# imisumi/software-path-tracer

Measured on AMD Instinct MI355X. Metric: Msamples/sec (whole node), 1920x1080 x 8-bounce Cornell box, higher is better.
Workload: dtype f32

## Files before the change

include/spt.h:

```cpp
#ifndef SPT_H
#define SPT_H

#include <stddef.h>
#include <stdint.h>

#ifdef __cplusplus
extern "C" {
#endif

#define SPT_ABI_VERSION 3

typedef enum spt_status {
    SPT_OK = 0,
    SPT_ERR_INVALID = -1,
    SPT_ERR_HIP = -2,
    SPT_ERR_NO_DEVICE = -3,
    SPT_ERR_NO_SCENE = -4,
    SPT_ERR_NOT_CONFIGURED = -5,
    SPT_ERR_CAPACITY = -6
} spt_status;


typedef enum spt_prim_type {
    SPT_PRIM_SPHERE = 0,
// ... 111 lines not shown
int spt_configure(spt_ctx* ctx, const spt_config* cfg);
int spt_reset(spt_ctx* ctx);
int spt_get_frame_count(const spt_ctx* ctx, uint32_t* frame_count);

int spt_render(spt_ctx* ctx, uint32_t first_frame, uint32_t n_frames);
int spt_synchronize(spt_ctx* ctx);

int spt_shard_pixels(const spt_ctx* ctx, uint64_t* n_pixels);
int spt_read_accum(spt_ctx* ctx, float* host_rgba);
int spt_accum_device_ptr(spt_ctx* ctx, void** dptr, size_t* bytes);
int spt_copy_accum_device(spt_ctx* ctx, void* dst);
int spt_resolve_rgba8(spt_ctx* ctx, uint32_t frame_count, uint32_t* host_out);
int spt_resolve_rgba8_exposure(spt_ctx* ctx, uint32_t frame_count, float exposure, uint32_t* host_out);
int spt_register_host_output(spt_ctx* ctx, void* host_out, size_t bytes);
int spt_render_resolve_rgba8(spt_ctx* ctx, uint32_t first_frame, uint32_t n_frames, uint32_t frame_count,
                             float exposure, uint32_t* host_out);
int spt_assemble_rows(spt_ctx* ctx, const void* gathered, void* out);

#define SPT_CAMERA_JITTER 1u
typedef struct spt_camera {
    float origin[3], u[3], v[3], w[3];
    uint32_t flags;
    uint32_t reserved[3];
} spt_camera;
int spt_set_camera(spt_ctx* ctx, const spt_camera* camera);
int spt_camera_look_at(const float eye[3], const float target[3], const float up[3], float vfov_degrees,
                       spt_camera* out);
int spt_camera_ray(const spt_camera* camera, uint32_t width, uint32_t height, uint32_t x, uint32_t y,
                   float jx, float jy, float o[3], float d[3]);

typedef struct spt_lens {
    float radius;
    float focus_distance;
    uint32_t reserved[2];
} spt_lens;
int spt_set_camera_lens(spt_ctx* ctx, const spt_lens* lens);
int spt_camera_lens_ray(const spt_camera* camera, const spt_lens* lens, uint32_t width, uint32_t height,
                        uint32_t x, uint32_t y, float jx, float jy, float u1, float u2, float o[3], float d[3]);
int spt_camera_focus_at_hit(const spt_camera* camera, uint32_t width, uint32_t height, uint32_t x, uint32_t y,
                            float jx, float jy, float t, float* focus_distance);

typedef enum spt_material_kind { SPT_MAT_DIFFUSE = 0, SPT_MAT_METAL = 1, SPT_MAT_DIELECTRIC = 2 } spt_material_kind;
typedef struct spt_material_model {
    uint32_t kind;
    float    param;
    uint32_t reserved[2];
} spt_material_model;
int spt_set_material_models(spt_ctx* ctx, const spt_material_model* models, uint32_t n);
int spt_bsdf_sample(const spt_material_model* model, const float d[3], const float n[3], int entering,
                    uint32_t flags, uint32_t* rng, float dir_out[3], int* transmitted, int* absorbed);

int spt_render_features(spt_ctx* ctx);
int spt_read_features(spt_ctx* ctx, float* feat_a, float* feat_b, float* albedo);
int spt_features_device_ptr(spt_ctx* ctx, void** feat_a, void** feat_b, void** albedo, size_t* bytes);

typedef struct spt_denoise_params {
    uint32_t levels;
    float    sigma_color;
    float    sigma_plane;
    uint32_t normal_power_log2;
    uint32_t reserved[4];
} spt_denoise_params;
int spt_denoise_params_default(spt_denoise_params* out);
int spt_denoise(spt_ctx* ctx, uint32_t frame_count, const spt_denoise_params* params);
int spt_set_denoise_form(spt_ctx* ctx, int form);
int spt_read_denoised(spt_ctx* ctx, float* host_rgba);
int spt_denoised_device_ptr(spt_ctx* ctx, void** dptr, size_t* bytes);
int spt_resolve_denoised_rgba8(spt_ctx* ctx, float exposure, uint32_t* host_out);
int spt_atrous_host(const float* rgba, const float* feat_a, const float* feat_b, uint32_t width, uint32_t height,
                    const spt_denoise_params* params, float* out);

int spt_set_env_map(spt_ctx* ctx, const float* rgba, uint32_t width, uint32_t height);
int spt_env_octa_from_equirect(const float* src_rgb, uint32_t src_width, uint32_t src_height, float* dst_rgba,
                               uint32_t dst_width, uint32_t dst_height);

enum spt_profile {
    SPT_PROFILE_EVENTS = 1,
    SPT_PROFILE_COUNTERS = 2,
    SPT_PROFILE_SPAN = 4
};
int spt_set_profiling(spt_ctx* ctx, int mode);
int spt_get_stats(spt_ctx* ctx, spt_stats* out);
int spt_stats_clear(spt_ctx* ctx);

#define SPT_COMM_ID_BYTES 128
int spt_comm_available(void);
int spt_comm_unique_id(uint8_t id[SPT_COMM_ID_BYTES]);
int spt_comm_init(spt_ctx* ctx, const uint8_t id[SPT_COMM_ID_BYTES], int n_ranks, int rank);
int spt_gather_image(spt_ctx* ctx, void* root_image);
int spt_gather_image_overlapped(spt_ctx* ctx, void* root_image);
int spt_gather_wait(spt_ctx* ctx);
int spt_comm_destroy(spt_ctx* ctx);

typedef struct spt_tuning {
    int32_t fused;
    uint32_t tail_bounce;
    int32_t persistent;
    int32_t frame_kernel;
    uint32_t chunks_per_wave;
    uint32_t px_shift;
    uint32_t subqueues;
    uint32_t bvh_max_leaf;
    uint32_t bvh_bins;
    int32_t specialize;
    int32_t view_cache;
    int32_t split_streams;
} spt_tuning;
int spt_set_tuning(spt_ctx* ctx, const spt_tuning* tuning);

int spt_specialize_scene(spt_ctx* ctx);
int spt_compile_flat_kernels(const spt_prim* prims, uint32_t n_prims, int env_map, char* log, size_t log_bytes);

typedef enum spt_scene_id {
    SPT_SCENE_C1_SPHERE_GROUND = 0,
    SPT_SCENE_APP_DEFAULT = 1,
    SPT_SCENE_CORNELL = 2,
    SPT_SCENE_BUNNYLIKE = 3,
    SPT_SCENE_INTERIOR_1M = 4
} spt_scene_id;
int spt_build_scene(uint32_t scene_id, spt_prim* prims, uint32_t* n_prims,
                    spt_material* mats, uint32_t* n_mats, spt_env* env);

#ifdef __cplusplus
}
#endif
#endif
```

software-path-tracer_amd/__init__.py:

```python
from __future__ import annotations

import ctypes
import enum
import os
from typing import Optional, Sequence, Tuple

import numpy as np

_HERE = os.path.dirname(os.path.abspath(__file__))
LIB_PATH = os.environ.get("SPT_LIB_PATH") or os.path.join(_HERE, "libspt_hip.so")
RENDER_LIB_PATH = os.path.join(_HERE, "libspt_render.so")

SPT_OK = 0
SPT_ERR = {
    -1: "SPT_ERR_INVALID",
    -2: "SPT_ERR_HIP",
    -3: "SPT_ERR_NO_DEVICE",
    -4: "SPT_ERR_NO_SCENE",
    -5: "SPT_ERR_NOT_CONFIGURED",
    -6: "SPT_ERR_CAPACITY",
}

PRIM_SPHERE, PRIM_QUAD, PRIM_TRIANGLE = 0, 1, 2
FLAG_ABS_FLOAT = 1
# ... 33 lines not shown
class SptEnv(ctypes.Structure):
    _fields_ = [("sky_enabled", ctypes.c_uint32), ("horizon", ctypes.c_float * 3), ("zenith", ctypes.c_float * 3)]


class SptConfig(ctypes.Structure):
    _fields_ = [
        ("width", ctypes.c_uint32),
        ("height", ctypes.c_uint32),
        ("max_bounces", ctypes.c_uint32),
        ("rr_depth", ctypes.c_uint32),
        ("flags", ctypes.c_uint32),
        ("shard_rank", ctypes.c_uint32),
        ("shard_count", ctypes.c_uint32),
        ("frames_in_flight", ctypes.c_uint32),
    ]


class SptCamera(ctypes.Structure):
    _fields_ = [
        ("origin", ctypes.c_float * 3),
        ("u", ctypes.c_float * 3),
        ("v", ctypes.c_float * 3),
        ("w", ctypes.c_float * 3),
        ("flags", ctypes.c_uint32),
        ("reserved", ctypes.c_uint32 * 3),
    ]


class SptLens(ctypes.Structure):
    _fields_ = [
        ("radius", ctypes.c_float),
        ("focus_distance", ctypes.c_float),
        ("reserved", ctypes.c_uint32 * 2),
    ]


CAMERA_JITTER = 1
SPT_MAX_BOUNCES = 32


class SptStats(ctypes.Structure):
    _fields_ = [
        ("frames", ctypes.c_uint64),
        ("paths", ctypes.c_uint64),
        ("segments", ctypes.c_uint64 * SPT_MAX_BOUNCES),
        ("segments_total", ctypes.c_uint64),
        ("passes", ctypes.c_uint64),
        ("extend_launches", ctypes.c_uint64),
        ("extend_ms", ctypes.c_double),
        ("extend_segments", ctypes.c_uint64),
        ("shade_launches", ctypes.c_uint64),
        ("shade_ms", ctypes.c_double),
        ("other_ms", ctypes.c_double),
        ("extend_ms_bounce", ctypes.c_double * SPT_MAX_BOUNCES),
        ("shade_ms_bounce", ctypes.c_double * SPT_MAX_BOUNCES),
        ("bvh_nodes", ctypes.c_uint64),
        ("scene_bytes", ctypes.c_uint64),
        ("radiance_updates", ctypes.c_uint64 * SPT_MAX_BOUNCES),
        ("tail_ms", ctypes.c_double),
        ("tail_launches", ctypes.c_uint64),
        ("tail_bounce", ctypes.c_uint64),
        ("fused", ctypes.c_uint64),
        ("persistent_ms", ctypes.c_double),
        ("persistent_launches", ctypes.c_uint64),
        ("schedule", ctypes.c_uint64),
        ("lane_slots", ctypes.c_uint64),
        ("lane_busy", ctypes.c_uint64),
        ("bvh_node_visits", ctypes.c_uint64),
        ("prim_tests", ctypes.c_uint64),
        ("flat_fast_path", ctypes.c_uint64),
        ("specialized", ctypes.c_uint64),
        ("shadow_rays", ctypes.c_uint64),
        ("emitters", ctypes.c_uint64),
        ("stack_bytes", ctypes.c_uint64),
        ("stack_need", ctypes.c_uint64),
        ("stalled_waves", ctypes.c_uint64),
        ("view_cached", ctypes.c_uint64),
        ("view_live_pixels", ctypes.c_uint64),
        ("flat_pairs", ctypes.c_uint64),
        ("flat_pair_second_passes", ctypes.c_uint64),
        ("view_split", ctypes.c_uint64),
        ("flat_sphere_second_passes", ctypes.c_uint64),
    ]

    def as_dict(self) -> dict:
        d = {}
        for k, _ in self._fields_:
            v = getattr(self, k)
            d[k] = list(v) if isinstance(v, ctypes.Array) else v
        return d


EXPORTED_SYMBOLS = (
    "spt_abi_version", "spt_device_count", "spt_create", "spt_destroy", "spt_last_error", "spt_set_stream",
    "spt_set_scene", "spt_configure", "spt_reset", "spt_get_frame_count", "spt_render", "spt_synchronize",
    "spt_shard_pixels", "spt_read_accum", "spt_accum_device_ptr", "spt_copy_accum_device", "spt_resolve_rgba8",
    "spt_resolve_rgba8_exposure", "spt_register_host_output", "spt_render_resolve_rgba8", "spt_assemble_rows",
    "spt_set_profiling", "spt_get_stats", "spt_stats_clear", "spt_build_scene",
    "spt_set_env_map", "spt_env_octa_from_equirect",
    "spt_comm_available", "spt_comm_unique_id", "spt_comm_init", "spt_gather_image", "spt_gather_image_overlapped", "spt_gather_wait",
    "spt_comm_destroy", "spt_set_tuning",
    "spt_specialize_scene", "spt_compile_flat_kernels", "spt_update_prims",
    "spt_set_camera", "spt_camera_look_at", "spt_camera_ray",
    "spt_set_camera_lens", "spt_camera_lens_ray", "spt_camera_focus_at_hit",
    "spt_set_material_models", "spt_bsdf_sample",
    "spt_render_features", "spt_read_features", "spt_features_device_ptr",
    "spt_denoise_params_default", "spt_denoise", "spt_set_denoise_form", "spt_read_denoised", "spt_denoised_device_ptr",
    "spt_resolve_denoised_rgba8", "spt_atrous_host",
)
COMM_ID_BYTES = 128


class SptTuning(ctypes.Structure):
    _fields_ = [
        ("fused", ctypes.c_int32),
        ("tail_bounce", ctypes.c_uint32),
        ("persistent", ctypes.c_int32),
        ("frame_kernel", ctypes.c_int32),
        ("chunks_per_wave", ctypes.c_uint32),
        ("px_shift", ctypes.c_uint32),
        ("subqueues", ctypes.c_uint32),
        ("bvh_max_leaf", ctypes.c_uint32),
        ("bvh_bins", ctypes.c_uint32),
        ("specialize", ctypes.c_int32),
        ("view_cache", ctypes.c_int32),
        ("split_streams", ctypes.c_int32),
    ]

    def __init__(self, **kw):
        super().__init__(fused=-1, persistent=-1, frame_kernel=-1)
        for k, v in kw.items():
            if k not in dict(self._fields_):
                raise TypeError(f"unknown spt_tuning field {k}")
            setattr(self, k, v)


class DenoiseParams(ctypes.Structure):
    _fields_ = [
        ("levels", ctypes.c_uint32),
        ("sigma_color", ctypes.c_float),
        ("sigma_plane", ctypes.c_float),
        ("normal_power_log2", ctypes.c_uint32),
        ("reserved", ctypes.c_uint32 * 4),
    ]

    def __init__(self, **kw):
        super().__init__()
        rc = load_library().spt_denoise_params_default(ctypes.byref(self))
        if rc != SPT_OK:
            raise SptError(f"spt_denoise_params_default -> {SPT_ERR.get(rc, rc)}")
        for k, v in kw.items():
            if k not in dict(self._fields_):
                raise TypeError(f"unknown spt_denoise_params field {k}")
            setattr(self, k, v)


_lib: Optional[ctypes.CDLL] = None


class SptError(RuntimeError):
    pass


def load_library(path: str = LIB_PATH) -> ctypes.CDLL:
    global _lib
    if _lib is not None:
        return _lib
    if not os.path.exists(path):
        raise SptError(f"libspt_hip.so not built at {path} (run `make` or __graft_entry__.build())")
    lib = ctypes.CDLL(path)
    P, U32, I = ctypes.c_void_p, ctypes.c_uint32, ctypes.c_int
    sig = {
        "spt_abi_version": ([], I),
        "spt_device_count": ([ctypes.POINTER(I)], I),
        "spt_create": ([ctypes.POINTER(P), I], I),
        "spt_destroy": ([P], None),
        "spt_last_error": ([P], ctypes.c_char_p),
        "spt_set_stream": ([P, P], I),
        "spt_set_scene": ([P, P, U32, P, U32, ctypes.POINTER(SptEnv)], I),
        "spt_configure": ([P, ctypes.POINTER(SptConfig)], I),
        "spt_reset": ([P], I),
        "spt_get_frame_count": ([P, ctypes.POINTER(U32)], I),
        "spt_render": ([P, U32, U32], I),
        "spt_synchronize": ([P], I),
        "spt_shard_pixels": ([P, ctypes.POINTER(ctypes.c_uint64)], I),
        "spt_read_accum": ([P, P], I),
        "spt_accum_device_ptr": ([P, ctypes.POINTER(P), ctypes.POINTER(ctypes.c_size_t)], I),
        "spt_copy_accum_device": ([P, P], I),
        "spt_resolve_rgba8": ([P, U32, P], I),
        "spt_resolve_rgba8_exposure": ([P, U32, ctypes.c_float, P], I),
        "spt_register_host_output": ([P, P, ctypes.c_size_t], I),
        "spt_render_resolve_rgba8": ([P, U32, U32, U32, ctypes.c_float, P], I),
        "spt_assemble_rows": ([P, P, P], I),
        "spt_set_profiling": ([P, I], I),
        "spt_set_env_map": ([P, P, U32, U32], I),
        "spt_env_octa_from_equirect": ([P, U32, U32, P, U32, U32], I),
        "spt_get_stats": ([P, ctypes.POINTER(SptStats)], I),
        "spt_stats_clear": ([P], I),
        "spt_build_scene": ([U32, P, ctypes.POINTER(U32), P, ctypes.POINTER(U32), ctypes.POINTER(SptEnv)], I),
        "spt_comm_available": ([], I),
        "spt_comm_unique_id": ([P], I),
        "spt_comm_init": ([P, P, I, I], I),
        "spt_gather_image": ([P, P], I),
        "spt_gather_image_overlapped": ([P, P], I),
        "spt_gather_wait": ([P], I),
        "spt_comm_destroy": ([P], I),
        "spt_set_tuning": ([P, ctypes.POINTER(SptTuning)], I),
        "spt_specialize_scene": ([P], I),
        "spt_update_prims": ([P, P, P, U32], I),
        "spt_compile_flat_kernels": ([P, U32, I, ctypes.c_char_p, ctypes.c_size_t], I),
        "spt_set_camera": ([P, ctypes.POINTER(SptCamera)], I),
        "spt_camera_look_at": ([ctypes.POINTER(ctypes.c_float), ctypes.POINTER(ctypes.c_float),
                                ctypes.POINTER(ctypes.c_float), ctypes.c_float, ctypes.POINTER(SptCamera)], I),
        "spt_camera_ray": ([ctypes.POINTER(SptCamera), U32, U32, U32, U32, ctypes.c_float, ctypes.c_float,
                            ctypes.POINTER(ctypes.c_float), ctypes.POINTER(ctypes.c_float)], I),
        "spt_set_camera_lens": ([P, ctypes.POINTER(SptLens)], I),
        "spt_camera_lens_ray": ([ctypes.POINTER(SptCamera), ctypes.POINTER(SptLens), U32, U32, U32, U32,
                                 ctypes.c_float, ctypes.c_float, ctypes.c_float, ctypes.c_float,
                                 ctypes.POINTER(ctypes.c_float), ctypes.POINTER(ctypes.c_float)], I),
        "spt_camera_focus_at_hit": ([ctypes.POINTER(SptCamera), U32, U32, U32, U32, ctypes.c_float, ctypes.c_float,
                                     ctypes.c_float, ctypes.POINTER(ctypes.c_float)], I),
        "spt_set_material_models": ([P, P, U32], I),
        "spt_bsdf_sample": ([P, ctypes.POINTER(ctypes.c_float), ctypes.POINTER(ctypes.c_float), I, U32,
                             ctypes.POINTER(U32), ctypes.POINTER(ctypes.c_float), ctypes.POINTER(I),
                             ctypes.POINTER(I)], I),
        "spt_render_features": ([P], I),
        "spt_read_features": ([P, P, P, P], I),
        "spt_features_device_ptr": ([P, ctypes.POINTER(P), ctypes.POINTER(P), ctypes.POINTER(P),
                                     ctypes.POINTER(ctypes.c_size_t)], I),
        "spt_denoise_params_default": ([ctypes.POINTER(DenoiseParams)], I),
        "spt_denoise": ([P, U32, ctypes.POINTER(DenoiseParams)], I),
        "spt_set_denoise_form": ([P, I], I),
        "spt_read_denoised": ([P, P], I),
        "spt_denoised_device_ptr": ([P, ctypes.POINTER(P), ctypes.POINTER(ctypes.c_size_t)], I),
        "spt_resolve_denoised_rgba8": ([P, ctypes.c_float, P], I),
        "spt_atrous_host": ([P, P, P, U32, U32, ctypes.POINTER(DenoiseParams), P], I),
    }
    for name, (args, res) in sig.items():
        if os.environ.get("SPT_LIB_PATH") and not hasattr(lib, name):
            continue
        fn = getattr(lib, name)
        fn.argtypes = args
        fn.restype = res
    _lib = lib
    return lib


def _ptr(a: np.ndarray) -> ctypes.c_void_p:
    return ctypes.c_void_p(a.ctypes.data) if a.size else ctypes.c_void_p(0)


def reference_env(sky: bool = True) -> SptEnv:
    e = SptEnv()
    e.sky_enabled = 1 if sky else 0
    e.horizon[:] = (1.0, 1.0, 1.0)
    e.zenith[:] = (0.5, 0.7, 1.0)
    return e


def env_octa_from_equirect(equirect_rgb: np.ndarray, width: int, height: int) -> np.ndarray:
    src = np.ascontiguousarray(equirect_rgb, dtype=np.float32)
    dst = np.zeros((height, width, 4), dtype=np.float32)
    rc = load_library().spt_env_octa_from_equirect(src.ctypes.data, src.shape[1], src.shape[0], dst.ctypes.data,
                                                   width, height)
    if rc != 0:
        raise SptError(f"spt_env_octa_from_equirect: {rc}")
    return dst


def synthetic_env_map(size: int = 512, seed: int = 0x5eed) -> np.ndarray:
    h, w = size // 2, size
    theta = (np.arange(h, dtype=np.float64) + 0.5) / h * np.pi
    phi = (np.arange(w, dtype=np.float64) + 0.5) / w * 2 * np.pi - np.pi
    th, ph = np.meshgrid(theta, phi, indexing="ij")
    y = np.cos(th)
    base = np.stack([0.6 + 0.4 * y, 0.7 + 0.3 * y, 1.0 + 0.2 * y], axis=-1)
    sun = np.exp(-((th - 0.6) ** 2 + (ph - 0.8) ** 2) / 0.002)[..., None] * np.array([40.0, 36.0, 30.0])
    ground = (y < 0)[..., None] * np.array([-0.3, -0.35, -0.5])
    noise = np.random.default_rng(seed).uniform(0.0, 0.05, size=(h, w, 1))
    equirect = np.maximum(base + sun + ground + noise, 0.0).astype(np.float32)
# ... 295 lines not shown
        self._env_keep = a
        self._check(self.lib.spt_set_env_map(self.h, a.ctypes.data, a.shape[1], a.shape[0]), "spt_set_env_map")

    def set_camera(self, cam: Optional[SptCamera]) -> None:
        self._check(self.lib.spt_set_camera(self.h, ctypes.byref(cam) if cam is not None else None), "spt_set_camera")
        self._camera = SptCamera.from_buffer_copy(cam) if cam is not None else None

    def set_camera_lens(self, radius=None, focus_distance: float = 1.0) -> None:
        if radius is None:
            self._check(self.lib.spt_set_camera_lens(self.h, None), "spt_set_camera_lens")
            return
        lens = _lens(radius, focus_distance)
        self._check(self.lib.spt_set_camera_lens(self.h, ctypes.byref(lens)), "spt_set_camera_lens")

    def focus_at(self, x: int, y: int) -> Optional[float]:
        if self._camera is None:
            raise SptError("focus_at needs a camera (set_camera)")
        w, h = self.width, self.height
        rank, count = int(self.cfg.shard_rank), max(1, int(self.cfg.shard_count))
        if not (0 <= x < w and 0 <= y < h) or y % count != rank:
            raise SptError("focus_at: the pixel is outside the image or on another ctx's rows")
        _, feat_b, _ = self.read_features()
        t = float(feat_b.reshape(-1, w, 4)[y // count, x, 3])
        if not np.isfinite(t):
            return None
        j = 0.5 if self._camera.flags & CAMERA_JITTER else 0.0
        return camera_focus_at_hit(self._camera, w, h, x, y, t, j, j)

    def set_material_models(self, models) -> None:
        if models is None:
            self._check(self.lib.spt_set_material_models(self.h, None, 0), "spt_set_material_models")
            return
        m = material_models(models)
        self._check(self.lib.spt_set_material_models(self.h, m.ctypes.data, len(m)), "spt_set_material_models")

    def render_features(self) -> None:
        self._check(self.lib.spt_render_features(self.h), "spt_render_features")

    def read_features(self) -> Tuple[np.ndarray, np.ndarray, np.ndarray]:
        n = self.shard_pixels
        a, b, alb = (np.zeros((n, 4), dtype=np.float32) for _ in range(3))
        self._check(self.lib.spt_read_features(self.h, _ptr(a), _ptr(b), _ptr(alb)), "spt_read_features")
        return a, b, alb

    def features_device_ptr(self) -> Tuple[int, int, int, int]:
        a, b, alb, n = ctypes.c_void_p(), ctypes.c_void_p(), ctypes.c_void_p(), ctypes.c_size_t()
        self._check(self.lib.spt_features_device_ptr(self.h, ctypes.byref(a), ctypes.byref(b), ctypes.byref(alb),
                                                     ctypes.byref(n)), "spt_features_device_ptr")
        return a.value or 0, b.value or 0, alb.value or 0, n.value

    def denoise(self, frame_count: int, params: Optional[DenoiseParams] = None) -> None:
        self._check(self.lib.spt_denoise(self.h, frame_count, ctypes.byref(params) if params is not None else None),
                    "spt_denoise")

    def set_denoise_form(self, form: int) -> None:
        self._check(self.lib.spt_set_denoise_form(self.h, form), "spt_set_denoise_form")

    def read_denoised(self) -> np.ndarray:
        out = np.zeros((self.shard_pixels, 4), dtype=np.float32)
        self._check(self.lib.spt_read_denoised(self.h, _ptr(out)), "spt_read_denoised")
        return out

    def denoised_device_ptr(self) -> Tuple[int, int]:
        p, n = ctypes.c_void_p(), ctypes.c_size_t()
        self._check(self.lib.spt_denoised_device_ptr(self.h, ctypes.byref(p), ctypes.byref(n)), "spt_denoised_device_ptr")
        return p.value or 0, n.value

    def resolve_denoised_rgba8(self, exposure: float = 1.0, out: Optional[np.ndarray] = None) -> np.ndarray:
        if out is None:
            out = np.zeros(self.shard_pixels, dtype=np.uint32)
        elif out.dtype != np.uint32 or not out.flags["C_CONTIGUOUS"] or out.size < self.shard_pixels:
            raise SptError("resolve_denoised_rgba8: out must be a C-contiguous uint32 array of >= shard_pixels")
        self._check(self.lib.spt_resolve_denoised_rgba8(self.h, exposure, _ptr(out)), "spt_resolve_denoised_rgba8")
        return out

    def set_profiling(self, enable, counters: bool = False, span: bool = False) -> None:
        mode = (PROFILE_EVENTS if enable and not span else 0) | (PROFILE_COUNTERS if counters else 0) | \
            (PROFILE_SPAN if span and enable else 0)
        self._check(self.lib.spt_set_profiling(self.h, mode), "spt_set_profiling")

    def stats(self) -> SptStats:
        s = SptStats()
        self._check(self.lib.spt_get_stats(self.h, ctypes.byref(s)), "spt_get_stats")
        return s

    def clear_stats(self) -> None:
        self._check(self.lib.spt_stats_clear(self.h), "spt_stats_clear")


def comm_available() -> bool:
    return load_library().spt_comm_available() == SPT_OK


def comm_unique_id() -> bytes:
    buf = ctypes.create_string_buffer(COMM_ID_BYTES)
    rc = load_library().spt_comm_unique_id(buf)
    if rc != SPT_OK:
        raise SptError(f"spt_comm_unique_id -> {SPT_ERR.get(rc, rc)}")
    return buf.raw


def device_count() -> int:
    lib = load_library()
    n = ctypes.c_int()
    lib.spt_device_count(ctypes.byref(n))
    return n.value


class BackendType(enum.IntEnum):

    CPU_EMBREE = 0
    GPU_OPTIX = 1
    GPU_METAL = 2
    GPU_HIP = 3


class RenderSettings:

    def __init__(self):
        self._width, self._height = 512, 512
        self._progressive = True
        self._spp, self._max_bounces, self._rr_depth = 64, 8, 3
        self._exposure = 1.0
        self._dirty = True

    def _set(self, name, value):
        if getattr(self, name) != value:
            setattr(self, name, value)
            self._dirty = True

    def setResolution(self, width: int, height: int) -> None:
        if (self._width, self._height) != (width, height):
            self._width, self._height = width, height
            self._dirty = True

    def setProgressive(self, v: bool) -> None:
        self._set("_progressive", v)

    def setSamplesPerPixel(self, v: int) -> None:
        self._set("_spp", v)

    def setMaxBounces(self, v: int) -> None:
        self._set("_max_bounces", v)

    def setRussianRouletteDepth(self, v: int) -> None:
        self._set("_rr_depth", v)

    def setExposure(self, v: float) -> None:
        self._set("_exposure", v)

    def getProgressive(self) -> bool:
        return self._progressive

    def getWidth(self) -> int:
        return self._width

    def getHeight(self) -> int:
        return self._height

    def getSamplesPerPixel(self) -> int:
        return self._spp

    def getMaxBounces(self) -> int:
        return self._max_bounces

    def getRussianRouletteDepth(self) -> int:
# ... 187 lines not shown
```

software-path-tracer_amd/csrc/spt_capi.hip:

```cpp
#include <dlfcn.h>
#include <hip/hip_runtime.h>
#include <rccl/rccl.h>

#include <algorithm>
#include <cmath>
#include <cstdio>
#include <cstdlib>
#include <cstring>
#include <string>
#include <vector>

#include "scene.h"
#include "spt.h"
#include "spt_denoise.h"
#include "spt_device.h"
#include "spt_jit.h"
#include "spt_kernels.h"
#include "spt_launch_plan.h"

using namespace spt;

static_assert(kBvhStackMax == kBvhStackEntries, "scene.h and spt_kernels.h stack bounds");
static_assert(kMatDiffuse == SPT_MAT_DIFFUSE && kMatMetal == SPT_MAT_METAL && kMatDielectric == SPT_MAT_DIELECTRIC,
              "spt.h spt_material_kind and spt_device.h model_kind");
static_assert(sizeof(spt_material_model) == 16, "spt_material_model is 16 bytes");
static_assert(sizeof(spt_denoise_params) == 32, "spt_denoise_params is 32 bytes");

namespace {

struct DevTree {
    std::vector<uint8_t> bytes;
    uint32_t stack_need = 0, stack_tb = 0;
};
template <int W, class Q, class QuantFn>
DevTree make_dev_tree(const std::vector<BvhNode>& bin, QuantFn quantize) {
    static_assert(sizeof(Q) == kDevNodeBytes, "device node record size");
    DevTree t;
    std::vector<BvhNodeW<W>> wide;
    collapse_bvh_w<W>(bin, wide);
    if (wide.empty()) return t;
    t.stack_need = bvh_w_stack_need<W>(wide, 0u);
    t.stack_tb = bvh_stack_t0_bits(bvh_w_max_ref<W>(wide));
    std::vector<Q> q;
    quantize(wide, q);
    t.bytes.resize(sizeof(Q) * q.size());
    std::memcpy(t.bytes.data(), q.data(), t.bytes.size());
    return t;
}
DevTree device_tree(const std::vector<BvhNode>& bin) { return make_dev_tree<4, BvhNodeQ>(bin, quantize_bvh4); }

struct EventPair {
    hipEvent_t a = nullptr, b = nullptr;
    int kind = 0;
    uint32_t bounce = 0;
    uint32_t launches = 1;
    hipEvent_t a2 = nullptr, b2 = nullptr;
};

struct ViewHalf {
    hipStream_t stream = nullptr;
    hipEvent_t done = nullptr;
    uint16_t* cost = nullptr;
    uint32_t* order = nullptr;
    uint64_t order_key = 0;
    uint32_t* work = nullptr;
    uint32_t work_parity = 0;
};

}

struct spt_ctx {
    int device = -1;
    hipStream_t own_stream = nullptr;
    hipStream_t user_stream = nullptr;
    ViewHalf half[2];
    hipEvent_t fork_ev = nullptr;
    bool stream_dirty = true;
    int32_t split_streams = 0;
    bool last_view_split = false;
    bool accum_shared = false;
    std::string err;
    uint32_t cu_count = 256;

    float4* d_prims = nullptr;
    float4* d_mats = nullptr;
    float4* d_nodes = nullptr;
    float4* d_env = nullptr;
    float4* d_emit = nullptr;
    uint32_t n_emit = 0;
    uint32_t n_emit_spheres = 0;
    uint32_t env_w = 0, env_h = 0;
    uint32_t n_prims = 0, n_nodes = 0, n_mats = 0;
    uint32_t n_dev_nodes = 0;
    void* bvh_stack = nullptr;
    uint32_t bvh_stack_need = 0;
    uint32_t bvh_stack_stride = 0;
    uint32_t bvh_stack_tb = 1;
    spt_env env{};
    bool has_scene = false;
    uint32_t flat_ends = 0;
    uint32_t flat_rect = 0;
    uint32_t flat_pairs = 0;
    bool fast_div = false;
    uint64_t scene_bytes = 0;
    uint64_t stack_bytes = 0;

    spt_config cfg{};
    bool configured = false;
    uint32_t rows = 0;
    uint32_t pixels = 0;
    uint32_t frames_per_pass = 1;
    uint32_t n_sub = 0;
    uint32_t sub_cap = 0;

    float4* q_o[2] = {nullptr, nullptr};
    float4* q_d[2] = {nullptr, nullptr};
    float4* q_t[2] = {nullptr, nullptr};
    float2* hit = nullptr;
    float4* radiance = nullptr;
    float4* accum = nullptr;
    float2* hit_cache = nullptr;
    bool hit_cache_valid = false;
    uint16_t* chunk_cost = nullptr;
    uint32_t* chunk_order = nullptr;
    uint64_t chunk_order_key = 0;
    float4* view_live = nullptr;
    float4* view_const = nullptr;
    uint32_t* view_counts = nullptr;
    uint32_t view_n[2] = {0, 0};
    bool view_valid = false;
    bool view_no_memory = false;
    int32_t view_cache = 0;
    bool last_view_cached = false;
    bool frame_lists = false;
    uint4* live_rec = nullptr;
    uint32_t* sky_pix = nullptr;
    uint32_t* list_counts = nullptr;
    uint32_t live_pixels = 0;
    uint32_t* counts = nullptr;
    unsigned long long* totals = nullptr;
    uint32_t* work = nullptr;
    uint32_t work_parity = 0;
    uint32_t chunks_per_wave = 0;
    uint32_t px_shift = 0;
    uint32_t* resolved = nullptr;
    void* out_host = nullptr;
    void* out_dev = nullptr;
    size_t out_bytes = 0;
    float fuse_frames = 0.0f, fuse_exposure = 1.0f;
    bool fused = false;

    uint32_t frame_count = 0;

    float4* feat_a = nullptr;
    float4* feat_b = nullptr;
    float4* feat_albedo = nullptr;
    bool feat_valid = false;
    uint32_t* d_mat_map = nullptr;
    float4* dn[2] = {nullptr, nullptr};
    int dn_result = -1;
    int dn_form = -1;

// ... 290 lines not shown
    if (!c->span_open) return SPT_OK;
    c->span_open = false;
    return end_event(c, c->span_ev);
}

bool schedule_fused(const spt_ctx* c) {
    if (c->cfg.flags & (SPT_FLAG_SPLIT_KERNELS | SPT_FLAG_SORTED_RAYS)) return false;
    if (c->fused_override >= 0) return c->fused_override != 0;
    return c->n_nodes == 0;
}

constexpr uint32_t kPersistentMaxFrames = 1024;

bool schedule_persistent(const spt_ctx* c, uint32_t n_frames) {
    if (c->cfg.max_bounces == 0) return false;
    if (c->cfg.flags & (SPT_FLAG_SPLIT_KERNELS | SPT_FLAG_WAVEFRONT | SPT_FLAG_SORTED_RAYS)) return false;
    if (c->persistent_override >= 0) return c->persistent_override != 0;
    return n_frames >= SPT_PERSISTENT_MIN_FRAMES;
}

bool schedule_frame(const spt_ctx* c) {
    if (c->cfg.max_bounces == 0) return false;
    if (c->cfg.flags & (SPT_FLAG_SPLIT_KERNELS | SPT_FLAG_WAVEFRONT | SPT_FLAG_SORTED_RAYS)) return false;
    if (c->frame_override >= 0) return c->frame_override != 0;
    if (c->persistent_override >= 0) return c->persistent_override != 0;
    return true;
}

uint32_t schedule_tail(const spt_ctx* c) {
    if (c->tail_override) return c->tail_override;
    return c->n_nodes == 0 ? 3u : kMaxBounces;
}

void next_work_set(spt_ctx* c, PassParams& p) {
    p.work = c->work + c->work_parity * kWorkWords;
    p.work_next = c->work + (c->work_parity ^ 1u) * kWorkWords;
    c->work_parity ^= 1u;
}

static uint64_t flat_jit_key(const spt_ctx* c) {
    const uint64_t shape = flat_shape_key(c->flat_ends, c->n_prims, c->flat_rect, c->flat_pairs);
    if (!c->configured) return shape;
    const uint32_t flags = (c->cfg.flags & ~spt::kFlagFastDiv) | (c->fast_div ? spt::kFlagFastDiv : 0u);
    return jit_config_key(shape, c->cfg.max_bounces, c->cfg.rr_depth, c->env.sky_enabled ? 1u : 0u, flags, c->has_camera);
}

static uint32_t sphere_emitters(const std::vector<DevEmitter>& emit) {
    uint32_t k = 0;
    for (const DevEmitter& e : emit) {
        uint32_t kind;
        std::memcpy(&kind, &e.base[3], 4);
        k += kind == 2u ? 1u : 0u;
    }
    return k;
}
static bool nee_active(const spt_ctx* c) { return c->configured && (c->cfg.flags & SPT_FLAG_NEE) && c->n_emit != 0u; }

static uint32_t camera_mode(const spt_ctx* c) {
    return ((c->camera.flags & SPT_CAMERA_JITTER) ? kCamJitter : kCamPosed) | (c->has_lens ? kCamLens : 0u);
}
static CameraLens lens_scalars(const spt_camera& cam, const spt_lens& lens) {
    auto len = [](const float v[3]) {
        return std::sqrt(((double)v[0] * v[0] + (double)v[1] * v[1]) + (double)v[2] * v[2]);
    };
    const double lu = len(cam.u), lv = len(cam.v);
    return CameraLens{lu > 0.0 ? (float)((double)lens.radius / lu) : 0.0f,
                      lv > 0.0 ? (float)((double)lens.radius / lv) : 0.0f, lens.focus_distance};
}
static int write_camera_record(spt_ctx* c) {
    SPT_HIP(c, hipSetDevice(c->device));
    SPT_HIP(c, hipStreamSynchronize(on_stream(c)));
    if (!c->d_camera) SPT_HIP(c, hipMalloc(&c->d_camera, 4 * sizeof(float4)));
    const spt_camera& cam = c->camera;
    const CameraLens l = c->has_lens ? lens_scalars(cam, c->lens) : CameraLens{0.0f, 0.0f, 0.0f};
    const uint32_t mode = camera_mode(c);
    float4 rec[4] = {make_float4(cam.origin[0], cam.origin[1], cam.origin[2], 0.0f),
                     make_float4(cam.u[0], cam.u[1], cam.u[2], l.a), make_float4(cam.v[0], cam.v[1], cam.v[2], l.b),
                     make_float4(cam.w[0], cam.w[1], cam.w[2], l.f)};
    std::memcpy(&rec[0].w, &mode, sizeof(mode));
    SPT_HIP(c, hipMemcpy(c->d_camera, rec, sizeof(rec), hipMemcpyHostToDevice));
    return SPT_OK;
}

static void prefetch_flat(const spt_ctx* c) {
    if (!(c->has_scene && c->configured && c->n_prims && c->n_nodes == 0 && c->specialize == 0)) return;
    const uint64_t key = flat_jit_key(c);
    const JitKindList kinds = jit_kinds_of_scene(nee_active(c), c->d_env ? 1 : 0);
    for (int i = 0; i < kinds.n; ++i) jit_prefetch(kinds.k[i].kind, kinds.k[i].env, key);
}

PassParams base_params(spt_ctx* c) {
    PassParams p{};
    p.prims = c->d_prims;
    p.mats = c->d_mats;
    p.nodes = c->d_nodes;
    p.n_prims = c->n_prims;
    p.n_mats = c->n_mats;
    p.n_nodes = c->n_nodes;
    p.n_dev_nodes = c->n_dev_nodes;
    p.sky_enabled = c->env.sky_enabled ? 1u : 0u;
    p.flags = (c->cfg.flags & ~spt::kFlagFastDiv) | (c->fast_div ? spt::kFlagFastDiv : 0u);
    p.flat_ends = c->flat_ends;
    for (int a = 0; a < 3; ++a) {
        p.bin_lo[a] = c->scene_lo[a];
        const float ext = c->scene_hi[a] - c->scene_lo[a];
        p.bin_scale[a] = ext > 0.0f ? 8.0f / ext : 0.0f;
    }
    p.ray_keys = c->ray_keys;
    p.ray_perm = c->ray_perm;
    p.ray_bins = c->ray_bins;
    p.ray_cursor = c->ray_cursor;
    p.jit_shape = (c->n_prims && c->n_nodes == 0 && c->specialize >= 0) ? flat_jit_key(c) : 0ull;
    p.jit_wait = c->specialize > 0 ? 1u : 0u;
    p.horizon = make_float4(c->env.horizon[0], c->env.horizon[1], c->env.horizon[2], 0.0f);
    p.zenith = make_float4(c->env.zenith[0], c->env.zenith[1], c->env.zenith[2], 0.0f);
    p.env = c->d_env;
    p.env_w = c->env_w;
    p.env_h = c->env_h;
    p.width = c->cfg.width;
    p.height = c->cfg.height;
    p.shard_rank = c->cfg.shard_rank;
    p.shard_count = c->cfg.shard_count;
    p.shard_pixels = c->pixels;
    p.inv_h = 1.0f / (float)c->cfg.height;
    p.inv_w = 1.0f / (float)c->cfg.width;
    p.aspect = (float)c->cfg.width / (float)c->cfg.height;
    p.max_bounces = c->cfg.max_bounces;
    p.rr_depth = c->cfg.rr_depth;
    p.n_sub = c->n_sub;
    p.sub_cap = c->sub_cap;
    for (int k = 0; k < 2; ++k) p.q[k] = QueueBufs{c->q_o[k], c->q_d[k], c->q_t[k]};
    p.hit = c->hit;
    p.radiance = c->radiance;
    p.accum = c->accum;
    p.counts = c->counts;
    p.totals = c->totals;
    p.cu_count = c->cu_count;
    p.chunks_per_wave = c->chunks_per_wave ? c->chunks_per_wave
                                           : ((c->n_nodes != 0 && c->n_prims <= 256u * 1024u) ? 4u : 2u);
    p.px_shift = c->px_shift;
    p.stack = c->bvh_stack;
    p.stack_need = c->bvh_stack_need;
    p.stack_stride = c->bvh_stack_stride;
    p.stack_tb = c->bvh_stack_tb;
    p.nee = NeeParams{c->d_emit, nee_active(c) ? c->n_emit : 0u, c->n_emit_spheres};
    if (c->has_camera) {
        p.cam_mode = camera_mode(c);
        p.cam_pose = c->d_camera;
    }
    p.bsdf = c->bsdf ? 1u : 0u;
    return p;
}

float model_word(const spt_material_model& m) {
    if (m.kind == SPT_MAT_METAL) return -std::fabs(m.param);
    return m.kind == SPT_MAT_DIELECTRIC ? m.param : 0.0f;
}
const char* model_error(const spt_material_model& m) {
    if (m.reserved[0] | m.reserved[1]) return "material model: reserved must be 0";
    if (!std::isfinite(m.param)) return "material model: non-finite parameter";
    if (m.kind == SPT_MAT_DIFFUSE) return m.param == 0.0f ? nullptr : "material model: a DIFFUSE parameter must be 0";
    if (m.kind == SPT_MAT_METAL) return m.param >= 0.0f && m.param <= 1.0f ? nullptr : "material model: fuzz outside [0, 1]";
    if (m.kind == SPT_MAT_DIELECTRIC) return m.param > 0.0f ? nullptr : "material model: index of refraction not > 0";
    return "material model: unknown kind";
}
int upload_materials(spt_ctx* c) {
    std::vector<DevMaterial> dm = c->h_dm;
    bool bsdf = false;
    if (!c->h_models.empty())
        for (size_t i = 0; i < dm.size(); ++i) {
// ... 390 lines not shown
        SPT_HIP(c, hipMalloc(&c->hit_cache, sizeof(float2) * std::max<size_t>(pixels, 1)));
        SPT_HIP(c, hipMalloc(&c->chunk_cost, sizeof(uint16_t) * std::max<size_t>(pixels, 1)));
        SPT_HIP(c, hipMalloc(&c->chunk_order, sizeof(uint32_t) * std::max<size_t>(pixels, 1)));
        if (kFrameHitCache >= 2) {
            SPT_HIP(c, hipMalloc(&c->live_rec, sizeof(uint4) * std::max<size_t>(pixels, 1)));
            SPT_HIP(c, hipMalloc(&c->sky_pix, sizeof(uint32_t) * std::max<size_t>(pixels, 1)));
            SPT_HIP(c, hipMalloc(&c->list_counts, sizeof(uint32_t) * (2 + (pixels + kBlock - 1) / kBlock)));
        }
        SPT_HIP(c, hipMalloc(&c->resolved, sizeof(uint32_t) * std::max<size_t>(pixels, 1)));
    }
    c->hit_cache_valid = false;
    c->feat_valid = false;
    c->dn_result = -1;
    c->chunk_order_key = 0;
    c->view_valid = false;
    const size_t qn = (size_t)cap * c->n_sub;
    if ((cfg->flags & SPT_FLAG_SORTED_RAYS) && qn && !c->ray_perm) {
        SPT_HIP(c, hipMalloc(&c->ray_keys, sizeof(uint16_t) * qn));
        SPT_HIP(c, hipMalloc(&c->ray_perm, sizeof(uint32_t) * qn));
        SPT_HIP(c, hipMalloc(&c->ray_bins, sizeof(uint32_t) * 4096));
        SPT_HIP(c, hipMalloc(&c->ray_cursor, sizeof(uint32_t) * 4097));
        SPT_HIP(c, hipMemset(c->ray_bins, 0, sizeof(uint32_t) * 4096));
    }
    c->configured = true;
    prefetch_flat(c);
    return spt_reset(c);
}

int spt_reset(spt_ctx* c) {
    if (!c) return SPT_ERR_INVALID;
    if (!c->configured) return fail(c, SPT_ERR_NOT_CONFIGURED, "spt_reset before spt_configure");
    SPT_HIP(c, hipSetDevice(c->device));
    SPT_HIP(c, hipMemsetAsync(c->accum, 0, sizeof(float4) * std::max<size_t>(c->pixels, 1), on_stream(c)));
    c->frame_count = 0;
    return SPT_OK;
}

int spt_get_frame_count(const spt_ctx* c, uint32_t* fc) {
    if (!c || !fc) return SPT_ERR_INVALID;
    *fc = c->frame_count;
    return SPT_OK;
}

static int build_view_lists(spt_ctx* c, const PassParams& p) {
    const size_t pixels = std::max<size_t>(c->pixels, 1);
    if (!c->view_live) {
        const size_t blocks = (pixels + kBlock - 1) / kBlock;
        if (hipMalloc(&c->view_live, sizeof(float4) * 3 * pixels) != hipSuccess ||
            hipMalloc(&c->view_const, sizeof(float4) * pixels) != hipSuccess ||
            hipMalloc(&c->view_counts, sizeof(uint32_t) * (2 + blocks)) != hipSuccess) {
            (void)hipGetLastError();
            free_dev(c->view_live);
            free_dev(c->view_const);
            free_dev(c->view_counts);
            c->view_no_memory = true;
            return SPT_OK;
        }
    }
    launch_view_lists(p, c->view_live, c->view_const, c->view_counts, c->view_counts + 2, on_stream(c));
    SPT_HIP(c, hipGetLastError());
    SPT_HIP(c, hipMemcpyAsync(c->view_n, c->view_counts, 2 * sizeof(uint32_t), hipMemcpyDeviceToHost, on_stream(c)));
    SPT_HIP(c, hipStreamSynchronize(on_stream(c)));
    c->view_valid = true;
    for (ViewHalf& h : c->half) h.order_key = 0;
    return SPT_OK;
}


static bool half_buffers(spt_ctx* c) {
    const size_t n = (size_t)c->pixels / 2u + 64u;
    for (ViewHalf& h : c->half) {
        if (h.cost && h.order) continue;
        if (hipMalloc(&h.cost, sizeof(uint16_t) * n) != hipSuccess || hipMalloc(&h.order, sizeof(uint32_t) * n) != hipSuccess) {
            (void)hipGetLastError();
            free_dev(h.cost);
            free_dev(h.order);
            return false;
        }
        h.order_key = 0;
    }
    return true;
}

static int launch_paths_split(spt_ctx* c, PassParams p, const ViewPlan& whole, bool launched[2]) {
    const ViewSplit sp = make_view_split(whole.n_live, whole.n_const, 1u << kMaxChunkShift);
    EventPair span_ev;
    if (c->profiling && c->span && begin_persistent(c, span_ev) != SPT_OK) return SPT_ERR_HIP;
    if (c->stream_dirty || c->accum_shared) {
        SPT_HIP(c, hipEventRecord(c->fork_ev, c->user_stream));
        for (ViewHalf& h : c->half) SPT_HIP(c, hipStreamWaitEvent(h.stream, c->fork_ev, 0));
        c->stream_dirty = false;
    }
    if (!c->chunks_per_wave) p.chunks_per_wave = 0u;
    const bool timed = c->profiling && !c->span;
    EventPair ev[2];
    int n_ev = 0;
    int rc = SPT_OK;
    for (uint32_t h = 0; h < 2u && rc == SPT_OK; ++h) {
        if (view_half_empty(sp, h)) continue;
        ViewHalf& vh = c->half[h];
        const ViewPlan view{whole.live + 3u * (size_t)sp.live_at[h], whole.constant + sp.const_at[h],
                            sp.live_at[h + 1] - sp.live_at[h], sp.const_at[h + 1] - sp.const_at[h], 0u};
        p.work = vh.work + vh.work_parity * kWorkWords;
        p.work_next = vh.work + (vh.work_parity ^ 1u) * kWorkWords;
        vh.work_parity ^= 1u;
        p.chunk_cost = vh.cost;
        p.chunk_order = vh.order;
        p.chunk_order_key = &vh.order_key;
        if (timed) {
            if (take_events(c, ev[n_ev], 4) != SPT_OK) return SPT_ERR_HIP;
            ++n_ev;
            if (hipEventRecord(ev[n_ev - 1].a, vh.stream) != hipSuccess) rc = fail(c, SPT_ERR_HIP, "k_paths (split): hipEventRecord");
        }
        c->last_specialized = launch_paths(p, c->counters, vh.stream, &view, h + 1u);
        launched[h] = true;
        const hipError_t le = hipGetLastError();
        if (le != hipSuccess) {
            vh.order_key = 0;
            rc = fail(c, SPT_ERR_HIP, std::string("k_paths (split): ") + hipGetErrorString(le));
        }
        if (timed && hipEventRecord(ev[n_ev - 1].b, vh.stream) != hipSuccess) rc = fail(c, SPT_ERR_HIP, "k_paths (split): hipEventRecord");
    }
    c->last_pairs = c->last_specialized ? flat_shape_pairs(p.jit_shape) : 0u;
    if (rc != SPT_OK) {
        for (int i = 0; i < n_ev; ++i) c->free_events.push_back(ev[i]);
        for (ViewHalf& h : c->half) h.order_key = 0;
        return rc;
    }
    if (n_ev) {
        if (n_ev == 2) {
            ev[0].a2 = ev[1].a;
            ev[0].b2 = ev[1].b;
        }
        c->pending.push_back(ev[0]);
        if (c->pending.size() >= 4096) return flush_events(c);
    }
    return SPT_OK;
}

static int join_halves(spt_ctx* c, bool launched[2]) {
    int rc = SPT_OK;
    for (uint32_t h = 0; h < 2u; ++h) {
        if (!launched[h]) continue;
        launched[h] = false;
        hipError_t e = hipEventRecord(c->half[h].done, c->half[h].stream);
        if (e == hipSuccess) e = hipStreamWaitEvent(c->user_stream, c->half[h].done, 0);
        if (e != hipSuccess) rc = fail(c, SPT_ERR_HIP, std::string("k_paths (split) join: ") + hipGetErrorString(e));
    }
    return rc;
}

static int render_persistent(spt_ctx* c, PassParams& p, uint32_t first_frame, uint32_t n_frames, bool launched[2]) {
    uint32_t done = 0;
    while (done < n_frames) {
        const uint32_t f = std::min(kPersistentMaxFrames, n_frames - done);
        p.first_frame = first_frame + done;
        p.n_frames = f;
        p.n_paths = f * c->pixels;
        const bool view_scene = c->view_cache >= 0 && view_lists_scene(p);
        const ViewPlan view{c->view_live, c->view_const, c->view_n[0], c->view_n[1], 0u};
        const bool view_on = view_scene && c->view_valid;
        if (view_on && split_call_wanted(c->split_streams, c->view_n[0], n_frames, kPersistentMaxFrames) && half_buffers(c)) {
            c->last_view_cached = c->last_view_split = true;
            const int rc = launch_paths_split(c, p, view, launched);
            if (rc != SPT_OK) return rc;
            done += f;
            c->passes++;
            continue;
        }
        if (join_halves(c, launched) != SPT_OK) return SPT_ERR_HIP;
        c->last_view_split = false;
        EventPair ev;
        if (begin_persistent(c, ev) != SPT_OK) return SPT_ERR_HIP;
        next_work_set(c, p);
        p.chunk_cost = c->chunk_cost;
        p.chunk_order = c->chunk_order;
        p.chunk_order_key = &c->chunk_order_key;
        c->last_specialized = launch_paths(p, c->counters, on_stream(c), view_on ? &view : nullptr);
        c->last_pairs = c->last_specialized ? flat_shape_pairs(p.jit_shape) : 0u;
        c->last_view_cached = view_on;
        const hipError_t le = hipGetLastError();
        if (le != hipSuccess) c->chunk_order_key = 0;
        if (end_persistent(c, ev) != SPT_OK) {
            c->chunk_order_key = 0;
            return SPT_ERR_HIP;
        }
        SPT_HIP(c, le);
        if (view_scene && !c->view_valid && !c->view_no_memory && build_view_lists(c, p) != SPT_OK) return SPT_ERR_HIP;
        done += f;
        c->passes++;
    }
    return SPT_OK;
}

int spt_render(spt_ctx* c, uint32_t first_frame, uint32_t n_frames) {
    if (!c) return SPT_ERR_INVALID;
    if (!c->has_scene) return fail(c, SPT_ERR_NO_SCENE, "Scene not set before rendering");
    if (!c->configured) return fail(c, SPT_ERR_NOT_CONFIGURED, "spt_render before spt_configure");
    if (c->sub_alloc != c->n_sub) return fail(c, SPT_ERR_NOT_CONFIGURED, "spt_set_tuning(subqueues) takes effect at spt_configure");
    SPT_HIP(c, hipSetDevice(c->device));
    if (c->pixels == 0 || n_frames == 0) {
        c->frame_count += n_frames;
        return SPT_OK;
    }
    PassParams p = base_params(c);
    uint32_t done = 0;
    if (schedule_persistent(c, n_frames)) {
        c->last_schedule = SPT_SCHEDULE_PERSISTENT;
        bool launched[2] = {false, false};
        const int rc = render_persistent(c, p, first_frame, n_frames, launched);
        const std::string err = c->err;
        const int joined = join_halves(c, launched);
        if (rc != SPT_OK) {
            c->err = err;
            return rc;
        }
        if (joined != SPT_OK) return joined;
        c->frames += n_frames;
        c->paths += (uint64_t)n_frames * c->pixels;
        c->frame_count += n_frames;
        return SPT_OK;
    }
    if (schedule_frame(c)) {
        c->last_schedule = SPT_SCHEDULE_FRAME;
        for (; done < n_frames; ++done) {
            p.first_frame = first_frame + done;
            p.n_frames = 1;
            p.n_paths = c->pixels;
            EventPair ev;
            if (begin_persistent(c, ev) != SPT_OK) return SPT_ERR_HIP;
            next_work_set(c, p);
            p.hit_cache = c->hit_cache;
            p.live_rec = c->live_rec;
            p.sky_pix = c->sky_pix;
            p.list_counts = c->list_counts;
            const bool jitter = cam_per_path(p.cam_mode) || p.bsdf != 0u;
            p.hit_mode = frame_hit_mode(p, c->hit_cache_valid, c->frame_lists);
            p.live_pixels = c->live_pixels;
            if (c->fuse_frames != 0.0f && done + 1u == n_frames) {
                p.rgba = (uint32_t*)c->out_dev;
                p.rgba_frames = c->fuse_frames;
                p.rgba_exposure = c->fuse_exposure;
                c->fused = true;
            }
            c->last_specialized = launch_frame(p, c->counters, on_stream(c));
            c->last_pairs = c->last_specialized ? flat_shape_pairs(p.jit_shape) : 0u;
            if (end_persistent(c, ev) != SPT_OK) return SPT_ERR_HIP;
            SPT_HIP(c, hipGetLastError());
            if (!c->hit_cache_valid) c->frame_lists = false;
            if (!jitter && !c->hit_cache_valid && frame_lists_scene(p, c->counters)) {
                launch_hit_lists(p, c->list_counts + 2, on_stream(c));
                SPT_HIP(c, hipGetLastError());
                SPT_HIP(c, hipMemcpyAsync(&c->live_pixels, c->list_counts, sizeof(uint32_t), hipMemcpyDeviceToHost,
                                          on_stream(c)));
                SPT_HIP(c, hipStreamSynchronize(on_stream(c)));
                c->frame_lists = c->pixels - c->live_pixels >= c->pixels / kFrameListsMinSkyDiv;
            }
            if (!jitter) c->hit_cache_valid = true;
            c->passes++;
        }
        c->frames += n_frames;
// ... 596 lines not shown
            float* o = dst + 4ull * ((size_t)iy * dw + ix);
            o[0] = t[0];
            o[1] = t[1];
            o[2] = t[2];
            o[3] = 1.0f;
        }
    }
    return SPT_OK;
}

int spt_set_profiling(spt_ctx* c, int mode) {
    if (!c) return SPT_ERR_INVALID;
    SPT_HIP(c, hipSetDevice(c->device));
    const bool span = (mode & SPT_PROFILE_SPAN) != 0;
    if (!span && close_span(c) != SPT_OK) return SPT_ERR_HIP;
    if (!(mode & (SPT_PROFILE_EVENTS | SPT_PROFILE_SPAN)) && flush_events(c) != SPT_OK) return SPT_ERR_HIP;
    c->profiling = (mode & (SPT_PROFILE_EVENTS | SPT_PROFILE_SPAN)) != 0;
    c->span = span;
    const bool counters = (mode & SPT_PROFILE_COUNTERS) != 0;
    if (counters != c->counters) c->hit_cache_valid = false;
    if (counters != c->counters) c->view_valid = false;
    c->counters = counters;
    return SPT_OK;
}

int spt_get_stats(spt_ctx* c, spt_stats* out) {
    if (!c || !out) return SPT_ERR_INVALID;
    SPT_HIP(c, hipSetDevice(c->device));
    SPT_HIP(c, hipStreamSynchronize(on_stream(c)));
    if (flush_events(c) != SPT_OK) return SPT_ERR_HIP;
    unsigned long long tot[kTotals];
    SPT_HIP(c, hipMemcpy(tot, c->totals, sizeof(tot), hipMemcpyDeviceToHost));
    std::memset(out, 0, sizeof(*out));
    out->frames = c->frames;
    out->paths = c->paths;
    out->passes = c->passes;
    for (uint32_t b = 0; b < kMaxBounces && b < SPT_MAX_BOUNCES; ++b) {
        out->segments[b] = tot[b];
        out->segments_total += tot[b];
        out->radiance_updates[b] = tot[kMaxBounces + b];
    }
    out->extend_launches = c->ext_launches;
    out->extend_ms = c->ext_ms;
    out->extend_segments = c->ext_launches ? out->segments_total : 0;
    out->shade_launches = c->shade_launches;
    out->shade_ms = c->shade_ms;
    out->other_ms = c->other_ms;
    out->tail_ms = c->tail_ms;
    out->tail_launches = c->tail_launches;
    out->tail_bounce = schedule_tail(c);
    out->fused = schedule_fused(c) ? 1u : 0u;
    out->persistent_ms = c->persist_ms;
    out->persistent_launches = c->persist_launches;
    out->schedule = c->last_schedule;
    out->lane_slots = tot[2 * kMaxBounces];
    out->lane_busy = tot[2 * kMaxBounces + 1];
    out->bvh_node_visits = tot[2 * kMaxBounces + 2];
    out->prim_tests = tot[2 * kMaxBounces + 3];
    out->flat_fast_path = (c->fast_div && c->n_prims <= kFlatSceneMax) ? 1u : 0u;
    out->specialized = c->last_specialized ? 1u : 0u;
    for (uint32_t b = 0; b < kMaxBounces && b < SPT_MAX_BOUNCES; ++b) {
        out->extend_ms_bounce[b] = c->ext_ms_b[b];
        out->shade_ms_bounce[b] = c->shade_ms_b[b];
    }
    out->bvh_nodes = c->n_nodes;
    out->scene_bytes = c->scene_bytes;
    out->shadow_rays = tot[kTotShadow];
    out->emitters = c->n_emit;
    out->stack_bytes = c->stack_bytes;
    out->stack_need = c->bvh_stack_need;
    out->stalled_waves = tot[kTotStalled];
    out->view_cached = c->last_view_cached ? 1u : 0u;
    out->view_live_pixels = c->view_valid ? c->view_n[0] : 0u;
    out->flat_pairs = c->last_specialized ? c->last_pairs : 0u;
    out->flat_pair_second_passes = tot[kTotPairSecond];
    out->flat_sphere_second_passes = tot[kTotSphereSecond];
    out->view_split = c->last_view_split ? 1u : 0u;
    if (tot[kTotStalled])
        return fail(c, SPT_ERR_HIP, "k_paths: " + std::to_string(tot[kTotStalled]) +
                                        " wave(s) stopped at the step bound with frames unaccumulated (a bug)");
    return SPT_OK;
}

int spt_stats_clear(spt_ctx* c) {
    if (!c) return SPT_ERR_INVALID;
    SPT_HIP(c, hipSetDevice(c->device));
    SPT_HIP(c, hipStreamSynchronize(on_stream(c)));
    if (flush_events(c) != SPT_OK) return SPT_ERR_HIP;
    SPT_HIP(c, hipMemset(c->totals, 0, sizeof(unsigned long long) * kTotals));
    c->frames = c->paths = c->passes = 0;
    c->ext_launches = c->shade_launches = c->ext_segments = 0;
    c->ext_ms = c->shade_ms = c->other_ms = c->tail_ms = 0.0;
    c->tail_launches = 0;
    c->persist_ms = 0.0;
    c->persist_launches = 0;
    for (uint32_t b = 0; b < kMaxBounces; ++b) c->ext_ms_b[b] = c->shade_ms_b[b] = 0.0;
    return SPT_OK;
}

int spt_specialize_scene(spt_ctx* c) {
    if (!c) return SPT_ERR_INVALID;
    if (!c->has_scene) return fail(c, SPT_ERR_NO_SCENE, "spt_specialize_scene before spt_set_scene");
    if (c->n_prims == 0 || c->n_nodes != 0 || c->specialize < 0) return SPT_OK;
    SPT_HIP(c, hipSetDevice(c->device));
    const uint64_t key = flat_jit_key(c);
    std::string err;
    const JitKindList kinds = jit_kinds_of_scene(nee_active(c), c->d_env ? 1 : 0);
    for (int i = 0; i < kinds.n; ++i)
        if (!jit_function(kinds.k[i].kind, kinds.k[i].env, key, &err))
            return fail(c, SPT_ERR_HIP, ("specialized kernels unavailable (the generic ones run): " + err).c_str());
    return SPT_OK;
}

int spt_compile_flat_kernels(const spt_prim* prims, uint32_t n_prims, int env_map, char* log, size_t log_bytes) {
    if (log && log_bytes) log[0] = 0;
    if ((!prims && n_prims) || n_prims == 0 || n_prims > kFlatSceneMax) return SPT_ERR_INVALID;
    uint32_t n_mats = 1;
    for (uint32_t i = 0; i < n_prims; ++i) n_mats = std::max(n_mats, prims[i].material + 1u);
    std::vector<DevPrim> dp, sorted;
    const char* msg = nullptr;
    if (!prepare_prims(prims, n_prims, n_mats, dp, &msg)) return SPT_ERR_INVALID;
    uint32_t ends[kFlatKinds - 1], flat_ends = 0;
    sort_flat_by_kind(dp, sorted, ends);
    for (uint32_t g = 0; g + 1 < kFlatKinds; ++g) flat_ends |= ends[g] << (6 * g);
    const uint32_t flat_rect = flat_rect_bits(sorted, ends);
    const uint64_t key = flat_shape_key(flat_ends, n_prims, flat_rect, flat_wall_pairs(sorted, ends, flat_rect));
    std::string out;
    const JitKindList kinds = jit_kinds_of_scene(false, env_map ? 1 : 0);
    int built = 0;
    while (built < kinds.n && jit_compile(kinds.k[built].kind, kinds.k[built].env, key, &out)) ++built;
    if (built == kinds.n) return SPT_OK;
    if (log && log_bytes) {
        std::strncpy(log, out.c_str(), log_bytes - 1);
        log[log_bytes - 1] = 0;
    }
    return SPT_ERR_HIP;
}

int spt_set_tuning(spt_ctx* c, const spt_tuning* t) {
    if (!c || !t) return SPT_ERR_INVALID;
    if (t->fused < -1 || t->fused > 1 || t->persistent < -1 || t->persistent > 1 || t->frame_kernel < -1 ||
        t->frame_kernel > 1)
        return fail(c, SPT_ERR_INVALID, "spt_tuning: fused / persistent / frame_kernel must be -1, 0 or 1");
    if (t->px_shift && (t->px_shift < 2 || t->px_shift > 5)) return fail(c, SPT_ERR_INVALID, "spt_tuning: px_shift 2..5");
    if (t->chunks_per_wave > 1024 || t->subqueues > 65536 || t->tail_bounce > kMaxBounces ||
        t->bvh_max_leaf > kBvhMaxLeaf || (t->bvh_bins && (t->bvh_bins < 2 || t->bvh_bins > 64)) ||
        t->specialize < -1 || t->specialize > 1 || t->view_cache < -1 || t->view_cache > 0 || t->split_streams < -1 ||
        t->split_streams > 1)
        return fail(c, SPT_ERR_INVALID, "spt_tuning: value out of range");
    SPT_HIP(c, hipSetDevice(c->device));
    SPT_HIP(c, hipStreamSynchronize(on_stream(c)));
    const uint32_t n_sub = t->subqueues ? t->subqueues : c->cu_count * 12u;
    if (n_sub != c->n_sub) {
        uint32_t* counts = nullptr;
        const size_t bytes = sizeof(uint32_t) * 2 * (kMaxBounces + 1) * n_sub;
        SPT_HIP(c, hipMalloc(&counts, bytes));
        if (hipMemset(counts, 0, bytes) != hipSuccess) {
            (void)hipFree(counts);
            return fail(c, SPT_ERR_HIP, "spt_set_tuning: hipMemset of the sub-queue counters failed");
        }
        free_dev(c->counts);
        c->counts = counts;
        c->n_sub = n_sub;
    }
    c->fused_override = t->fused;
    c->tail_override = t->tail_bounce;
    c->persistent_override = t->persistent;
    c->frame_override = t->frame_kernel;
    c->chunks_per_wave = t->chunks_per_wave;
    c->px_shift = t->px_shift;
    c->bvh_max_leaf = t->bvh_max_leaf;
    c->bvh_bins = t->bvh_bins;
    c->specialize = t->specialize;
    c->view_cache = t->view_cache;
    c->split_streams = t->split_streams;
    return SPT_OK;
}

int spt_comm_available(void) { return rccl().ok ? SPT_OK : SPT_ERR_NO_DEVICE; }

int spt_comm_unique_id(uint8_t id[SPT_COMM_ID_BYTES]) {
    static_assert(sizeof(ncclUniqueId) == SPT_COMM_ID_BYTES, "RCCL unique id size");
    if (!id) return SPT_ERR_INVALID;
    if (!rccl().ok) return SPT_ERR_NO_DEVICE;
    ncclUniqueId u;
    if (rccl().get_unique_id(&u) != ncclSuccess) return SPT_ERR_HIP;
    std::memcpy(id, &u, sizeof(u));
    return SPT_OK;
}

int spt_comm_init(spt_ctx* c, const uint8_t id[SPT_COMM_ID_BYTES], int n_ranks, int rank) {
    if (!c || !id) return SPT_ERR_INVALID;
    if (n_ranks < 1 || rank < 0 || rank >= n_ranks) return fail(c, SPT_ERR_INVALID, "spt_comm_init: rank out of range");
    if (!rccl().ok) return fail(c, SPT_ERR_NO_DEVICE, rccl().err);
    SPT_HIP(c, hipSetDevice(c->device));
    SPT_HIP(c, hipStreamSynchronize(on_stream(c)));
    free_comm(c);
    ncclUniqueId u;
    std::memcpy(&u, id, sizeof(u));
    SPT_NCCL(c, rccl().comm_init_rank(&c->comm, n_ranks, u, rank));
    c->comm_ranks = n_ranks;
    c->comm_rank = rank;
    return SPT_OK;
}

int spt_comm_destroy(spt_ctx* c) {
    if (!c) return SPT_ERR_INVALID;
    SPT_HIP(c, hipSetDevice(c->device));
    SPT_HIP(c, hipStreamSynchronize(on_stream(c)));
    free_comm(c);
    return SPT_OK;
}

namespace {
int gather_check(spt_ctx* c, void* root_image, const char* what, uint32_t& rows_max, size_t& shard_elems) {
    if (!c->configured) return fail(c, SPT_ERR_NOT_CONFIGURED, "not configured");
    if (!c->comm) return fail(c, SPT_ERR_INVALID, std::string(what) + " before spt_comm_init");
    const uint32_t world = c->cfg.shard_count;
    if ((int)world != c->comm_ranks || (int)c->cfg.shard_rank != c->comm_rank)
        return fail(c, SPT_ERR_INVALID, std::string(what) + ": shard_rank / shard_count differ from the communicator's rank / size");
    if (c->comm_rank == 0 && !root_image) return fail(c, SPT_ERR_INVALID, std::string(what) + ": rank 0 needs an output image");
    SPT_HIP(c, hipSetDevice(c->device));
    rows_max = (c->cfg.height + world - 1) / world;
    shard_elems = (size_t)rows_max * c->cfg.width * 4;
    return SPT_OK;
}

int gather_buffer(spt_ctx* c, size_t need) {
    if (c->gather_elems == need) return SPT_OK;
    if (c->gather_pending) SPT_HIP(c, hipStreamWaitEvent(on_stream(c), c->gather_done, 0));
    SPT_HIP(c, hipStreamSynchronize(on_stream(c)));
    free_dev(c->gather_buf);
    if (need) {
        SPT_HIP(c, hipMalloc(&c->gather_buf, sizeof(float) * need));
        SPT_HIP(c, hipMemsetAsync(c->gather_buf, 0, sizeof(float) * need, on_stream(c)));
    }
    c->gather_elems = need;
    return SPT_OK;
}
}

int spt_gather_image(spt_ctx* c, void* root_image) {
    if (!c) return SPT_ERR_INVALID;
    uint32_t rows_max = 0;
    size_t shard_elems = 0;
    int st = gather_check(c, root_image, "spt_gather_image", rows_max, shard_elems);
    if (st != SPT_OK) return st;
    const bool root = c->comm_rank == 0;
    const bool padded = c->rows < rows_max;
    st = gather_buffer(c, root ? shard_elems * c->cfg.shard_count : (padded ? shard_elems : 0));
    if (st != SPT_OK) return st;
    if (c->gather_pending) SPT_HIP(c, hipStreamWaitEvent(on_stream(c), c->gather_done, 0));
    const float4* send = c->accum;
    if (padded && !root) {
        if (c->pixels)
            SPT_HIP(c, hipMemcpyAsync(c->gather_buf, c->accum, sizeof(float4) * c->pixels, hipMemcpyDeviceToDevice, on_stream(c)));
        send = c->gather_buf;
    }
// ... 51 lines not shown
```

software-path-tracer_amd/csrc/spt_jit.h:

```cpp
#pragma once

#include <hip/hip_runtime.h>
#include <stdint.h>

#include <string>
#include <vector>

namespace spt {

enum : int { kJitPaths, kJitFrame, kJitPathsChan, kJitPathsNee, kJitFrameNee, kJitFrameRgba, kJitFrameNeeRgba,
             kJitPathsStats, kJitPathsNeeStats, kJitKinds };
constexpr int kJitCallersEnv = -1;
struct JitKindRow {
    const char* kernel;
    const char* tail;
    int env;
    bool stats;
};
constexpr JitKindRow kJitKindTable[kJitKinds] = {
    {"k_paths", "", kJitCallersEnv},
    {"k_frame", "", kJitCallersEnv},
    {"k_paths", ", 0, true", kJitCallersEnv},
    {"k_paths", ", 0, false, 1", 2},
    {"k_frame", ", false, 1", 2},
    {"k_frame", ", false, 0, true", kJitCallersEnv},
    {"k_frame", ", false, 1, true", 2},
    {"k_paths", "", kJitCallersEnv, true},
    {"k_paths", ", 0, false, 1", 2, true},
};
inline std::string jit_name_expr(int kind, int env, uint64_t shape) {
    const JitKindRow& k = kJitKindTable[kind];
    return std::string("spt::") + k.kernel + (k.stats ? "<true, false, " : "<false, false, ") +
           std::to_string(k.env == kJitCallersEnv ? env : k.env) + ", " + std::to_string((unsigned long long)shape) + "ull" + k.tail + ">";
}

bool jit_compile(int kernel, int env, uint64_t shape, std::string* log, std::vector<char>* code = nullptr);
std::string jit_compiler();
hipFunction_t jit_function(int kernel, int env, uint64_t shape, std::string* err, bool wait = true);
void jit_prefetch(int kernel, int env, uint64_t shape);
bool jit_ready(int kernel, int env, uint64_t shape);

}
```

software-path-tracer_amd/csrc/spt_kernels.h:

```cpp
#pragma once

#ifndef __HIPCC_RTC__
#include <hip/hip_runtime.h>
#include <stdint.h>
#endif

namespace spt {

constexpr uint32_t kBlock = 256;
constexpr uint32_t kChunk = 64;
constexpr uint32_t kMaxBounces = 32;
constexpr uint32_t kFlagFastDiv = 1u << 30;
constexpr uint32_t kTotShadow = 2 * kMaxBounces + 4;
constexpr uint32_t kTotStalled = 2 * kMaxBounces + 5;
constexpr uint32_t kTotPairSecond = 2 * kMaxBounces + 6;
constexpr uint32_t kTotSphereSecond = 2 * kMaxBounces + 7;
constexpr uint32_t kOnePassMax = 4;
constexpr uint32_t kTotals = 2 * kMaxBounces + 8;

constexpr uint32_t kFlagNee = 1u << 4;
struct NeeParams {
    const float4* emit;
    uint32_t n_emit;
    uint32_t spheres;
// ... 59 lines not shown
    uint32_t hit_mode;
    const uint4* live_rec;
    const uint32_t* sky_pix;
    const uint32_t* list_counts;
    uint32_t live_pixels;
    uint32_t* rgba;
    float rgba_frames, rgba_exposure;
    uint16_t* chunk_cost;
    uint32_t* chunk_order;
    uint64_t* chunk_order_key;
    uint32_t cam_mode;
    uint32_t bsdf;
    const float4* cam_pose;
};

constexpr uint32_t kCamReference = 0;
constexpr uint32_t kCamPosed = 1;
constexpr uint32_t kCamJitter = 2;
constexpr uint32_t kCamLens = 4;
__host__ __device__ constexpr bool cam_per_path(uint32_t cam_mode) { return (cam_mode & (kCamJitter | kCamLens)) != 0u; }

constexpr uint64_t kShapeValid = 1ull << 36;
__host__ __device__ constexpr uint64_t flat_shape_key(uint32_t flat_ends, uint32_t n_prims, uint32_t rect_bits = 0u,
                                                      uint32_t pair_bits = 0u) {
    return kShapeValid | (uint64_t)(n_prims & 63u) << 30 | (flat_ends & 0x3fffffffu) | (uint64_t)(rect_bits & 7u) << 53 |
           (uint64_t)(pair_bits & 63u) << 57;
}
__host__ __device__ constexpr uint32_t flat_shape_pairs(uint64_t key, uint32_t ax) {
    return (uint32_t)(key >> (57u + 2u * ax)) & 3u;
}
__host__ __device__ constexpr uint32_t flat_shape_pairs(uint64_t key) {
    return flat_shape_pairs(key, 0u) + flat_shape_pairs(key, 1u) + flat_shape_pairs(key, 2u);
}
__host__ __device__ constexpr uint32_t flat_pair_table_bytes(uint64_t key) {
    return flat_shape_pairs(key) ? 64u * flat_shape_pairs(key) + 16u : 0u;
}
constexpr uint64_t kConfigValid = 1ull << 37;
constexpr uint32_t kFlagAbsFloatBit = 1u;
constexpr uint64_t kConfigCamera = 1ull << 56;
__host__ __device__ constexpr uint64_t jit_config_key(uint64_t shape, uint32_t max_bounces, uint32_t rr_depth,
                                                      uint32_t sky_enabled, uint32_t flags, bool camera = false) {
    if (max_bounces > 63u || rr_depth > 63u) return shape;
    return shape | kConfigValid | (uint64_t)max_bounces << 38 | (uint64_t)rr_depth << 44 |
           (uint64_t)(sky_enabled != 0u) << 50 | (uint64_t)((flags & kFlagAbsFloatBit) != 0u) << 51 |
           (uint64_t)((flags & kFlagFastDiv) != 0u) << 52 | (camera ? kConfigCamera : 0ull);
}

constexpr uint32_t kBvhStackEntry = 4;
constexpr uint32_t kBvhStackEntry8W = 8;
constexpr uint32_t kBvhStackEntryBytes = kBvhStackEntry > kBvhStackEntry8W ? kBvhStackEntry : kBvhStackEntry8W;
inline __host__ __device__ constexpr uint32_t bvh_stack_t0_bits(uint32_t max_ref) {
    uint32_t rb = 0;
    while (rb < 32u && (max_ref >> rb) != 0u) ++rb;
    const uint32_t tb = 32u - rb;
    return tb > 28u ? 28u : tb;
}
struct StackCode {
    uint32_t sh, base, mask;
};
inline __host__ __device__ constexpr StackCode stack_code_params(uint32_t tb) {
    return StackCode{28u - tb, 0x3a800000u >> (28u - tb), (1u << tb) - 1u};
}
inline __host__ __device__ constexpr uint32_t stack_code(uint32_t t0_bits, StackCode c) {
    const uint32_t q = (t0_bits >> c.sh) - c.base;
    return q < c.mask ? q : c.mask;
}
inline __host__ __device__ constexpr uint32_t stack_t0_lower_bits(uint32_t code, StackCode c) {
    return ((code & c.mask) + c.base) << c.sh;
}
constexpr uint32_t kBvhStackEntries = 96;
inline __host__ __device__ constexpr uint32_t bvh_stack_stride(uint32_t need) { return need < 1u ? 1u : (need + 3u) & ~3u; }
constexpr uint32_t kMaxResidentWaves = 8 * 4;
constexpr uint32_t kDevNodeBytes = 64u;

constexpr uint32_t kFrameHitCache = 2;
constexpr uint32_t kFrameListsMinSkyDiv = 4;

constexpr int kBvhSmallWaves = 8;
constexpr uint32_t kFrameTopPrims = 64;
constexpr uint32_t kFrameTopNodes = 64;
constexpr uint32_t kBvhSmall = 256u * 1024u;
constexpr uint32_t kMaxChunkShift = 5;
constexpr uint32_t kMinChunkShift = 0;

struct ChunkPlan {
    uint32_t n[3];
    uint32_t start[3];
    uint32_t shift[3];
    const uint32_t* order;
    uint16_t* cost;
};

constexpr uint32_t kViewSweep = 64;
struct ViewPlan {
    const float4* live;
    const float4* constant;
    uint32_t n_live, n_const;
    uint32_t n_sweep;
};

constexpr uint32_t kFrameRun = 128;
constexpr uint32_t kFrameRunBvh = 64;
constexpr uint32_t kFrameLdsStackMax = 16;
__host__ __device__ constexpr uint32_t frame_chunk(bool bvh) { return bvh ? kFrameRunBvh : kFrameRun; }
constexpr int kFrameWavesSmall = 5;
constexpr uint32_t kFrameSkyPerLane = 4;

constexpr uint32_t kWorkHeads = 8;
constexpr uint32_t kWorkStride = 32;
constexpr uint32_t kWorkWords = kWorkHeads * kWorkStride;

#ifndef __HIPCC_RTC__
void launch_extend(const PassParams& p, uint32_t bounce, hipStream_t s);
void launch_extend_sorted(const PassParams& p, uint32_t bounce, hipStream_t s);
void launch_shade(const PassParams& p, uint32_t bounce, hipStream_t s);
void launch_bounce(const PassParams& p, uint32_t bounce, hipStream_t s);
void launch_trace_tail(const PassParams& p, uint32_t bounce, hipStream_t s);
void launch_accumulate(const PassParams& p, hipStream_t s);
bool launch_paths(const PassParams& p, bool stats, hipStream_t s, const ViewPlan* view = nullptr,
                  uint32_t view_half = 0u);
inline bool view_lists_scene(const PassParams& p) {
    return p.nodes == nullptr && p.n_prims != 0u && !cam_per_path(p.cam_mode) && p.bsdf == 0u;
}
void launch_view_lists(const PassParams& p, float4* live, float4* constant, uint32_t* counts, uint32_t* block_scratch,
                       hipStream_t s);
bool launch_frame(const PassParams& p, bool stats, hipStream_t s);
inline bool frame_small_scene(const PassParams& p, bool stats) {
    return p.nodes != nullptr && !stats && p.nee.n_emit == 0u && p.n_dev_nodes <= kFrameTopNodes &&
           p.n_prims <= kFrameTopPrims && 4u * p.n_prims + 2u * p.n_mats <= 4u * kFrameTopPrims &&
           p.stack_need <= kFrameLdsStackMax;
}
inline bool frame_small_scene_lists(const PassParams& p) {
    return p.shard_pixels / kFrameRunBvh > (uint32_t)kFrameWavesSmall * 4u * p.cu_count;
}
inline bool frame_lists_scene(const PassParams& p, bool stats) {
    if (kFrameHitCache < 2) return false;
    if (frame_small_scene(p, stats)) return frame_small_scene_lists(p);
    return true;
}
void launch_hit_lists(const PassParams& p, uint32_t* block_scratch, hipStream_t s);
void launch_resolve(const float4* accum, uint32_t n, float frames, float exposure, uint32_t* out, hipStream_t s);
void launch_assemble_rows(const float4* gathered, float4* out, uint32_t width, uint32_t height,
                          uint32_t world, uint32_t rows_max, hipStream_t s);

#endif

inline __host__ __device__ uint32_t deal_sub(uint32_t p, uint32_t n_sub) { return (p / kChunk) % n_sub; }
inline __host__ __device__ uint32_t deal_slot(uint32_t p, uint32_t n_sub) {
    return (p / (kChunk * n_sub)) * kChunk + (p % kChunk);
}
inline __host__ __device__ uint32_t dealt_path(uint32_t s, uint32_t i, uint32_t n_sub) {
    return ((i / kChunk) * n_sub + s) * kChunk + (i % kChunk);
}
inline __host__ __device__ uint32_t sub_count_of(uint32_t n, uint32_t s, uint32_t n_sub) {
    const uint32_t per_round = kChunk * n_sub;
    const uint32_t full = (n / per_round) * kChunk;
    const uint32_t rem = n % per_round;
    const uint32_t lo = s * kChunk;
    const uint32_t extra = rem > lo ? (rem - lo < kChunk ? rem - lo : kChunk) : 0u;
    return full + extra;
}
inline uint32_t sub_capacity(uint64_t n_paths, uint32_t n_sub) {
    const uint64_t per_round = (uint64_t)kChunk * n_sub;
    return (uint32_t)(((n_paths + per_round - 1) / per_round) * kChunk);
}

}
```

software-path-tracer_amd/csrc/spt_kernels.hip:

```cpp
#ifndef __HIPCC_RTC__
#include <algorithm>
#endif

#include "spt_device.h"
#include "spt_kernels.h"

namespace spt {

namespace {

__device__ __forceinline__ float isect_any(const float4* __restrict__ prims, uint32_t k, uint32_t type, F3 o, F3 d) {
    if (type == 0u) return isect_sphere(prims[4 * k + 0], o, d, kTNear);
    if (type == 1u) return isect_quad(prims[4 * k + 0], prims[4 * k + 1], prims[4 * k + 2], prims[4 * k + 3], o, d, kTNear);
    return isect_tri(prims[4 * k + 0], prims[4 * k + 1], prims[4 * k + 2], o, d, kTNear);
}

__device__ __forceinline__ void closest_flat_exact(const float4* __restrict__ prims, uint32_t n_prims, F3 o, F3 d,
                                                   float& best_t, uint32_t& best_k) {
    for (uint32_t k = 0; k < n_prims; ++k) {
        const float t = isect_any(prims, k, meta_type(prims[4 * k + 3]), o, d);
        if (t < best_t) {
            best_t = t;
            best_k = k;
        }
// ... 1153 lines not shown
constexpr uint32_t kFlatPxRecs = 3;
constexpr int kPathsWaves = 6;
constexpr int kPathsWavesFlat = 7;
constexpr int kPathsWavesBvh = 7;
constexpr uint32_t kBvhTopNodes = 53;
constexpr uint32_t kBvhTopNodes8 = 5;

#ifdef SPT_STATIC_PROFILE
#define SPT_MARK(x) asm volatile("; SPT_MARK " #x)
#else
#define SPT_MARK(x) ((void)0)
#endif

__device__ __forceinline__ float add_count(float w, uint32_t k) {
    if (w + (float)k <= 16777216.0f) return w + (float)k;
    for (uint32_t i = 0; i < k; ++i) w = w + 1.0f;
    return w;
}
__device__ __forceinline__ float add_frames(float a, uint32_t c, float v, uint32_t n) {
    if (c == 3u) return add_count(a, n);
    for (uint32_t f = 0; f < n; ++f) a = a + v;
    return a;
}

__device__ __forceinline__ uint32_t lane_id_here() {
    uint32_t v;
    asm volatile("v_mbcnt_lo_u32_b32 %0, -1, 0\n\tv_mbcnt_hi_u32_b32 %0, -1, %0" : "=v"(v));
    return v;
}

__device__ __forceinline__ uint32_t xcc_id() {
    uint32_t v;
    asm volatile("s_getreg_b32 %0, hwreg(HW_REG_XCC_ID, 0, 4)" : "=s"(v));
    return v;
}

__device__ __forceinline__ uint32_t pull_unit(uint32_t* __restrict__ work, uint32_t n, uint32_t xcc, uint32_t& h) {
    while (h < kWorkHeads) {
        const uint32_t r = (xcc + h) & (kWorkHeads - 1u);
        const uint32_t len = n > r ? (n - r + kWorkHeads - 1u) / kWorkHeads : 0u;
        uint32_t k = len;
        if (__lane_id() == 0u) {
            uint32_t* head = work + r * kWorkStride;
            if (h == 0u || __hip_atomic_load(head, __ATOMIC_RELAXED, __HIP_MEMORY_SCOPE_AGENT) < len)
                k = atomicAdd(head, 1u);
        }
        k = __builtin_amdgcn_readfirstlane(k);
        if (k < len) return r + k * kWorkHeads;
        ++h;
    }
    return n;
}

#ifdef SPT_TIMELINE
__device__ unsigned long long g_tl[8192 * 4];
#endif

constexpr uint32_t kBvhBatch = 24;
constexpr uint32_t kBvhBatchNee = 48;

template <bool kStats, bool kLds = false, bool kAnyHit = false, class Stk>
__device__ __forceinline__ void advance_rays(const float4* __restrict__ nodes, const float4* __restrict__ prims,
                                             bool have, bool can_start, F3 o, F3 d, Trav& tv, bool& tdone,
                                             const Stk& stk, BvhCounters& ctr,
                                             uint32_t& lane_slots, uint32_t& lane_busy,
                                             const float4* top = nullptr, uint32_t n_top = 0u,
                                             const float4* ptop = nullptr, uint32_t n_ptop = 0u,
                                             uint32_t batch = kBvhBatch) {
    for (;;) {
        const bool trav = have && !tdone;
        const unsigned long long tm = __ballot(trav);
        if (tm == 0ull) break;
        if ((uint32_t)__popcll(__ballot(have ? tdone : can_start)) >= batch) break;
        if (kStats) {
            lane_slots += 64u;
            lane_busy += (uint32_t)__popcll(tm);
        }
        if (trav)
            tdone = trav_step<kStats, kLds, kAnyHit>(nodes, prims, o, d, tv, stk, &ctr, top, n_top, ptop, n_ptop);
    }
}

template <bool kStats, bool kBvh, int kEnv, uint64_t kShape = 0, int kSimdWaves = 0, bool kChan = false, int kNee = 0,
          bool kJitter = false, bool kBsdf = false>
__global__ __launch_bounds__(kBlock, kSimdWaves ? kSimdWaves : (kBvh ? kPathsWavesBvh : ((kNee || kBsdf) ? kPathsWaves : kPathsWavesFlat))) void k_paths(const float4* __restrict__ prims, const float4* __restrict__ mats,
                                                  const float4* __restrict__ nodes, uint32_t n_prims,
                                                  float4* __restrict__ accum,
                                                  unsigned long long* __restrict__ totals,
                                                  uint32_t* __restrict__ work, uint32_t* __restrict__ work_next,
                                                  ShadeParams sp, CameraParams cam, uint32_t n_frames, ChunkPlan plan,
                                                  NeeParams nee, ViewPlan view) {
    constexpr uint32_t kWaves = kBlock / 64u;
    constexpr bool kStart0 = kJitter || kBsdf;
    constexpr bool kView = !kBvh && !kStart0;
    bake_config<kShape>(sp);
    constexpr uint32_t kRingSlots = ring_slots<kBvh>();
    extern __shared__ float4 s_scene[];
    constexpr uint32_t kPxRecs = kBvh ? 3u : kFlatPxRecs;
    __shared__ float4 s_px[kWaves][kPxRecs][1u << kMaxChunkShift];
    __shared__ float s_L[kWaves][3][kRingSlots];
    __shared__ __attribute__((aligned(16))) uint32_t s_cnt[kWaves][64];
    __shared__ uint8_t s_pix[kWaves][1u << kMaxChunkShift];
    constexpr uint32_t kTop = kBvh ? (kSimdWaves == 8 ? kBvhTopNodes8 : kBvhTopNodes) : 0u;
    __shared__ float4 s_top[kTop ? 4u * kTop : 1u];
    const uint32_t n_top = min(kTop, sp.n_nodes);
    for (uint32_t k = threadIdx.x; k < 4u * n_top; k += kBlock) s_top[k] = nodes[k];
    __shared__ uint32_t s_seg[kStats ? kMaxBounces : 1u];
    __shared__ uint32_t s_rmw[kStats ? kMaxBounces : 1u];
    __shared__ uint32_t s_shadow[kStats && kNee ? 1u : 1u];
    if (kStats && kNee && threadIdx.x == 0u) s_shadow[0] = 0u;
    if (!kBvh) make_shade_recs(prims, mats, sp.n_prims, s_scene);
    constexpr uint32_t kPairs = kBvh ? 0u : flat_shape_pairs(kShape);
    [[maybe_unused]] float4* const pair_tab = s_scene + 3u * ((uint32_t)(kShape >> 30) & 63u);
    [[maybe_unused]] uint32_t* const pair_second = kStats ? (uint32_t*)(pair_tab + 4u * kPairs) : nullptr;
    constexpr bool kCountSpheres = kStats && kPairs != 0u && (kShape & 63u) >= 2u && (kShape & 63u) <= kOnePassMax;
    if constexpr (kPairs != 0u) {
        make_pair_table<kShape>(prims, pair_tab);
        if (kStats && threadIdx.x == 0u) *pair_second = 0u;
        if (kCountSpheres && threadIdx.x == 0u) pair_second[1] = 0u;
    }
    if (blockIdx.x == 0u && threadIdx.x < kWorkHeads) work_next[threadIdx.x * kWorkStride] = 0u;
    if (kStats && threadIdx.x < kMaxBounces) {
        s_seg[threadIdx.x] = 0;
        s_rmw[threadIdx.x] = 0;
    }
    __syncthreads();
    const float4* sh_prims = kBvh ? prims : s_scene;
    const float4* sh_mats = mats;

    const uint32_t wave = __builtin_amdgcn_readfirstlane(threadIdx.x / 64u);
    const uint32_t lane = __lane_id();
    const auto stk = lane_stack<kSimdWaves == 8 ? kBvhStackEntry8W : kBvhStackEntry>(sp, blockIdx.x * kWaves + wave, lane);
    uint32_t lane_slots = 0, lane_busy = 0;
    BvhCounters bvh_ctr;
    uint32_t n_chunks = plan.n[0] + plan.n[1] + plan.n[2];
    bool view_on = false;
    if constexpr (kView) {
        view_on = view.live != nullptr;
        if (view_on) n_chunks += view.n_sweep;
    }
    const uint32_t xcc = xcc_id();
    uint32_t heads_empty = 0;
    constexpr bool kOrdered = true;
#ifdef SPT_TIMELINE
    const unsigned long long tl_start = wall_clock64();
    unsigned long long tl_last = tl_start;
    uint32_t tl_chunks = 0, tl_pxs = 0, tl_live = 0;
#endif
    for (;;) {
        uint32_t chunk = pull_unit(work, n_chunks, xcc, heads_empty);
        if (chunk >= n_chunks) break;
#ifdef SPT_TIMELINE
        tl_last = wall_clock64();
        ++tl_chunks;
#endif
        if constexpr (kView) {
            if (view_on && chunk >= plan.n[0]) {
                const uint32_t unit = chunk - plan.n[0];
                if (unit < view.n_sweep) {
                    const uint32_t i0 = unit * kViewSweep;
                    if (kStats && lane == 0u) atomicAdd(&s_seg[0], n_frames * min(kViewSweep, view.n_const - i0));
                    if (i0 + lane < view.n_const) {
                        const float4 c = view.constant[i0 + lane];
                        const uint32_t pix = __float_as_uint(c.w);
                        float4 a = accum[pix];
                        for (uint32_t f = 0; f < n_frames; ++f) a = make_float4(a.x + c.x, a.y + c.y, a.z + c.z, a.w);
                        a.w = add_count(a.w, n_frames);
                        accum[pix] = a;
                    }
#ifdef SPT_TIMELINE
                    tl_pxs = 6u;
                    tl_live = 0u;
#endif
                    continue;
                }
                chunk -= view.n_sweep;
            }
        }
        uint32_t pxs, pix0;
        if (chunk < plan.n[0]) {
            pxs = plan.shift[0];
            pix0 = ((kOrdered && plan.order) ? __builtin_amdgcn_readfirstlane(plan.order[chunk]) : chunk) << pxs;
        } else if (chunk < plan.n[0] + plan.n[1]) {
            pxs = plan.shift[1];
            pix0 = plan.start[1] + ((chunk - plan.n[0]) << pxs);
        } else {
            pxs = plan.shift[2];
            pix0 = plan.start[2] + ((chunk - plan.n[0] - plan.n[1]) << pxs);
        }
        const uint32_t px = 1u << pxs;
        const uint32_t npx = min(px, ((kView && view_on) ? view.n_live : cam.shard_pixels) - pix0);
        constexpr bool chmode = kBvh || kChan;
        const uint32_t cp = lane & (px - 1u);
        const uint32_t c0 = pxs == kMaxChunkShift ? 2u * (lane >> pxs) : (lane >> pxs);
        const bool ch_on = chmode && c0 < 4u && cp < npx;
        float4 acc = make_float4(0.f, 0.f, 0.f, 0.f);
        bool live_px = false;
        PrimaryState ps;
        uint32_t apix = pix0 + (chmode ? cp : lane);
        if constexpr (kView) {
            if (view_on) {
                uint32_t vpix = 0;
                if (lane < npx) {
                    const float4* rec = view.live + 3u * (size_t)(pix0 + lane);
                    ps.r0 = rec[0];
                    ps.r1 = rec[1];
                    ps.r2 = rec[2];
                    vpix = __float_as_uint(ps.r2.w);
                    live_px = true;
                }
                apix = chmode ? (uint32_t)__shfl((int)vpix, (int)cp, 64) : vpix;
            }
        }
        if (ch_on) {
            const float* af = reinterpret_cast<const float*>(accum) + 4u * (size_t)apix + c0;
            acc.x = af[0];
            if (pxs == kMaxChunkShift) acc.y = af[1];
        }
        if (lane < npx) {
            if (!chmode) acc = accum[apix];
            if (!(kView && view_on)) {
                const uint32_t pix = pix0 + lane;
                const uint32_t lrow = pix / cam.width;
                const uint32_t x = pix - lrow * cam.width;
                const uint32_t y = cam.shard_rank + cam.shard_count * lrow;
                if constexpr (kStart0) {
                    ps.r0 = make_float4(__uint_as_float(x), __uint_as_float(y), 0.f, __uint_as_float(x + y * cam.width));
                    ps.r1 = ps.r2 = make_float4(0.f, 0.f, 0.f, 0.f);
                    live_px = true;
                } else {
                    const CameraRay cr = camera_ray_xy<kShape, false>(cam, x, y, x + y * cam.width);
                    ps = primary_state<kBvh, kEnv, kShape>(prims, nodes, n_prims, prims, mats, sp, cr.o, cr.d, cr.seed, stk);
                    live_px = (__float_as_uint(ps.r1.w) & kHitBit) != 0u && 1u < sp.max_bounces;
                }
            }
        }
        F3 lc{ps.r1.x, ps.r1.y, ps.r1.z};
        if (!live_px && lane < npx && (__float_as_uint(ps.r1.w) & kHitBit)) {
            if (!kBvh) {
                lc = F3{ps.r4.x, ps.r4.y, ps.r4.z};
            } else {
                const float4 emi = sh_mats[2u * (__float_as_uint(ps.r1.w) & ~kHitBit) + 1u];
                lc = emi.w != 0.0f ? F3{0.0f + 1.0f * emi.x, 0.0f + 1.0f * emi.y, 0.0f + 1.0f * emi.z}
                                   : F3{0.f, 0.f, 0.f};
            }
        }
        if (kStats && !kStart0 && lane == 0u) atomicAdd(&s_seg[0], n_frames * npx);
        const uint32_t live_mask = (uint32_t)__ballot(live_px);
        const uint32_t n_live = (uint32_t)__popc(live_mask);
#ifdef SPT_TIMELINE
        tl_pxs = pxs;
        tl_live = n_live;
#endif
        if (kOrdered && plan.cost && n_live == 0u && chunk < plan.n[0] && lane == 0u) plan.cost[chunk] = 0u;
        if (n_live == 0u) {
            const float lx = __shfl(lc.x, (int)cp, 64), ly = __shfl(lc.y, (int)cp, 64), lz = __shfl(lc.z, (int)cp, 64);
            const float v0 = c0 == 0u ? lx : (c0 == 1u ? ly : lz);
            const float v1 = c0 + 1u == 1u ? ly : lz;
            if (ch_on) {
                acc.x = add_frames(acc.x, c0, v0, n_frames);
                if (pxs == kMaxChunkShift) acc.y = add_frames(acc.y, c0 + 1u, v1, n_frames);
                float* af = reinterpret_cast<float*>(accum) + 4u * (size_t)(pix0 + cp) + c0;
                af[0] = acc.x;
                if (pxs == kMaxChunkShift) af[1] = acc.y;
            } else if (!chmode && lane < npx) {
                for (uint32_t f = 0; f < n_frames; ++f) acc = make_float4(acc.x + lc.x, acc.y + lc.y, acc.z + lc.z, acc.w + 1.0f);
                accum[pix0 + lane] = acc;
            }
            continue;
        }
        const uint32_t li = __builtin_amdgcn_mbcnt_lo(live_mask, 0u);
        if (live_px) {
            s_px[wave][0][li] = ps.r0;
            s_px[wave][1][li] = ps.r1;
            s_px[wave][2][li] = ps.r2;
        } else if (lane < npx) {
            s_px[wave][0][n_live + lane - li] = make_float4(lc.x, lc.y, lc.z, 0.f);
        }
        if (lane < px) s_pix[wave][lane] = (uint8_t)(live_px ? li : (kConstPx | (n_live + lane - li)));
        s_cnt[wave][lane] = 0;
        uint8_t* const ring_flg = reinterpret_cast<uint8_t*>(&s_cnt[wave][0]);
        const uint32_t m_live = __builtin_amdgcn_readfirstlane((0x80000000u + n_live - 1u) / n_live);
        auto div_live = [&](uint32_t s) { return __umulhi(s << 1, m_live); };
        constexpr bool kPixRing = kChan;
        const uint32_t sr_sh = kPixRing ? 8u - (32u - (uint32_t)__builtin_clz(2u * n_live - 1u) - 1u) : 0u;
        const uint32_t win = kPixRing ? (n_live << sr_sh) : kRingSlots;
        auto ring_entry = [&](uint32_t s) {
            if (!kPixRing) return s & (kRingSlots - 1u);
            const uint32_t f = div_live(s);
            return ((s - f * n_live) << sr_sh) | (f & ((1u << sr_sh) - 1u));
        };
        __builtin_amdgcn_fence(__ATOMIC_RELEASE, "wavefront");
        __builtin_amdgcn_wave_barrier();
        __builtin_amdgcn_fence(__ATOMIC_ACQUIRE, "wavefront");

        uint32_t q = 0;
        bool have = false;
        F3 o{0.f, 0.f, 0.f}, d{0.f, 0.f, 0.f}, T{1.f, 1.f, 1.f}, L{0.f, 0.f, 0.f};
        uint32_t rng = 0, bc = 0;
        Trav tv;
        bool tdone = false;
        constexpr bool kInline = kNee && !kBvh;
        bool shadow = false, after = false;
        bool spec = false;
        float smax = 0.f;
        F3 nd{0.f, 0.f, 0.f};

        const uint32_t n_slots = n_frames * n_live;
        uint32_t next = 0;
        uint32_t oldest_s = 0;

        auto finish = [&](bool fin) {
            if (fin) {
                const uint32_t e = ring_entry(q);
                s_L[wave][0][e] = L.x;
                s_L[wave][1][e] = L.y;
                s_L[wave][2][e] = L.z;
                ring_flg[q & (kRingSlots - 1u)] = (uint8_t)((q / kRingSlots) + 1u);
            }
        };
        auto accumulate = [&]() {
            __builtin_amdgcn_fence(__ATOMIC_RELEASE, "wavefront");
            __builtin_amdgcn_wave_barrier();
            __builtin_amdgcn_fence(__ATOMIC_ACQUIRE, "wavefront");
            const uint32_t base = oldest_s & ~3u;
            const uint32_t a = base + 4u * lane_id_here();
            const uint32_t want = ((a / kRingSlots) + 1u) * 0x01010101u;
            const uint32_t w = reinterpret_cast<const uint32_t*>(ring_flg)[(a & (kRingSlots - 1u)) >> 2];
            const uint32_t keep = a == base ? ~0u << (8u * (oldest_s & 3u)) : ~0u;
            const uint32_t miss = (w ^ want) & keep;
            const unsigned long long full = __ballot(miss == 0u);
            const uint32_t dz = ~full == 0ull ? 64u : (uint32_t)__builtin_ctzll(~full);
            uint32_t run = 4u * dz;
            if (dz < 64u)
                run += (uint32_t)__builtin_ctz((uint32_t)__builtin_amdgcn_readlane((int)miss, (int)dz)) >> 3;
            const uint32_t k = min(div_live(n_slots - oldest_s), div_live(run - (oldest_s & 3u)));
            if (k == 0u) return;
            if (ch_on) {
                const uint32_t ix = s_pix[wave][cp];
                const bool lv = ix < kConstPx;
                const float* cl = reinterpret_cast<const float*>(&s_px[wave][0][ix & ((1u << kMaxChunkShift) - 1u)]);
                const uint32_t c1 = c0 + 1u;
                const bool two = pxs == kMaxChunkShift && c1 < 3u;
                const float k0 = c0 < 3u ? cl[c0 < 3u ? c0 : 0u] : 0.f, k1 = cl[c1 < 3u ? c1 : 0u];
                if (kPixRing && c0 < 3u) {
                    const uint32_t msk = (1u << sr_sh) - 1u;
                    const uint32_t j0 = div_live(oldest_s) & msk;
                    const uint32_t n1 = min(k, msk + 1u - j0);
                    const float* pr = &s_L[wave][c0 < 3u ? c0 : 0u][(lv ? ix : 0u) << sr_sh];
                    auto run = [&](const float* p, uint32_t n) {
                        uint32_t f = 0;
                        for (; f + 4u <= n; f += 4u) {
                            const float x0 = p[f], x1 = p[f + 1u], x2 = p[f + 2u], x3 = p[f + 3u];
                            asm volatile("" ::"v"(x0), "v"(x1), "v"(x2), "v"(x3));
                            acc.x = (((acc.x + (lv ? x0 : k0)) + (lv ? x1 : k0)) + (lv ? x2 : k0)) + (lv ? x3 : k0);
                        }
                        for (; f < n; ++f) {
                            const float x0 = p[f];
                            asm volatile("" ::"v"(x0));
                            acc.x = acc.x + (lv ? x0 : k0);
                        }
                    };
                    run(pr + j0, n1);
                    run(pr, k - n1);
                } else if (c0 < 3u) {
                    const float* r0 = &s_L[wave][c0 < 3u ? c0 : 0u][0];
                    const float* r1 = &s_L[wave][c1 < 3u ? c1 : 0u][0];
                    uint32_t e = oldest_s + ix;
                    uint32_t f = 0;
                    for (; f + 2u <= k; f += 2u) {
                        const uint32_t e0 = e & (kRingSlots - 1u), e1 = (e + n_live) & (kRingSlots - 1u);
                        e += 2u * n_live;
                        const float x0 = lv ? r0[e0] : k0, x1 = lv ? r0[e1] : k0;
                        acc.x = (acc.x + x0) + x1;
                        if (two) {
                            const float y0 = lv ? r1[e0] : k1, y1 = lv ? r1[e1] : k1;
                            acc.y = (acc.y + y0) + y1;
                        }
                    }
                    if (f < k) {
                        const uint32_t e0 = e & (kRingSlots - 1u);
                        acc.x = acc.x + (lv ? r0[e0] : k0);
                        if (two) acc.y = acc.y + (lv ? r1[e0] : k1);
                    }
                } else {
                    acc.x = add_count(acc.x, k);
                }
                if (pxs == kMaxChunkShift && c1 == 3u) acc.y = add_count(acc.y, k);
            } else if (!chmode && lane < npx) {
                const uint32_t ix = s_pix[wave][lane];
                const bool lv = ix < kConstPx;
                const float4 c = s_px[wave][0][ix & ((1u << kMaxChunkShift) - 1u)];
                uint32_t e = oldest_s + ix;
                uint32_t f = 0;
                for (; f + 2u <= k; f += 2u) {
                    const uint32_t e0 = e & (kRingSlots - 1u), e1 = (e + n_live) & (kRingSlots - 1u);
                    e += 2u * n_live;
                    const float x0 = lv ? s_L[wave][0][e0] : c.x, y0 = lv ? s_L[wave][1][e0] : c.y,
                                z0 = lv ? s_L[wave][2][e0] : c.z;
                    const float x1 = lv ? s_L[wave][0][e1] : c.x, y1 = lv ? s_L[wave][1][e1] : c.y,
                                z1 = lv ? s_L[wave][2][e1] : c.z;
                    acc.x = (acc.x + x0) + x1;
                    acc.y = (acc.y + y0) + y1;
                    acc.z = (acc.z + z0) + z1;
                    acc.w = (acc.w + 1.0f) + 1.0f;
                }
                if (f < k) {
                    const uint32_t e0 = e & (kRingSlots - 1u);
                    acc.x = acc.x + (lv ? s_L[wave][0][e0] : c.x);
                    acc.y = acc.y + (lv ? s_L[wave][1][e0] : c.y);
                    acc.z = acc.z + (lv ? s_L[wave][2][e0] : c.z);
                    acc.w = acc.w + 1.0f;
                }
            }
            oldest_s += k * n_live;
            __builtin_amdgcn_fence(__ATOMIC_RELEASE, "wavefront");
            __builtin_amdgcn_wave_barrier();
            __builtin_amdgcn_fence(__ATOMIC_ACQUIRE, "wavefront");
        };

// ... 105 lines not shown
                                    if (kBvh) {
                                        trav_init(tv, d);
                                        tdone = false;
                                    }
                                } else {
                                    have = false;
                                    fin = true;
                                }
                            } else if (alive) {
                                if (kBsdf) spec = false;
                                o = offset_origin(o, n);
                                nee_hit(n, fin);
                                if (pend) dt = bounce_tangent(n, sp.flags);
                            }
                        }
                    } else {
                    bool alive;
                    F3 add;
                    ModelHit mh{0u, true, false};
                    SPT_MARK(shade);
                    const bool contributes =
                        shade_hit<kEnv, !kBvh, false, kBsdf>(sh_prims, sh_mats, sp, bc + 1u, best_t, best_k, o, d, T, rng, alive, add, dn, &mh);
                    bool scattered = false;
                    if constexpr (kBsdf) {
                        if (alive && mh.word != 0u) {
                            scattered = alive = scatter_specular<true>(mh, dn, sp.flags, o, d, rng);
                            if (kBvh && alive) {
                                trav_init(tv, d);
                                tdone = false;
                            }
                        } else if (alive) {
                            o = offset_origin(o, dn);
                        }
                    }
                    if (alive && !scattered) {
                        dt = bounce_tangent(dn, sp.flags);
                        pend = true;
                    }
                    if (contributes) L = F3{L.x + add.x, L.y + add.y, L.z + add.z};
                    if (kStats) {
                        atomicAdd(&s_seg[bc], 1u);
                        if (contributes) atomicAdd(&s_rmw[bc], 1u);
                    }
                    ++bc;
                    fin = !alive;
                    have = alive;
                    }
                }
                finish(fin);
            }
            SPT_MARK(acc_check);
            if (next + 64u > min(n_slots, oldest_s + win)) accumulate();
            SPT_MARK(handout);
            const bool idle = !have;
            const unsigned long long m = __ballot(idle);
            const uint32_t rank =
                __builtin_amdgcn_mbcnt_hi((uint32_t)(m >> 32), __builtin_amdgcn_mbcnt_lo((uint32_t)m, 0u));
            const uint32_t limit = min(n_slots, oldest_s + win);
            bool fin0 = false;
            const bool take = idle && next + rank < limit;
            if (take) {
                q = next + rank;
                const uint32_t f = div_live(q);
                const uint32_t r = q - f * n_live;
                const uint32_t frame = cam.first_frame + f + 1u;
                const float4 p0 = s_px[wave][0][r];
                if constexpr (kStart0) {
                    rng = rng_seed(__float_as_uint(p0.w), 0u, 0u, frame);
                    const CameraRay cr = camera_ray_xy<0>(cam, __float_as_uint(p0.x), __float_as_uint(p0.y), rng);
                    o = cr.o;
                    d = cr.d;
                    rng = cr.seed;
                    if constexpr (kBsdf) spec = false;
                    T = F3{1.f, 1.f, 1.f};
                    L = F3{0.f, 0.f, 0.f};
                    bc = 0u;
                    have = true;
                    if (kBvh) {
                        trav_init(tv, d);
                        tdone = false;
                    }
                } else {
                const float4 p1 = s_px[wave][1][r];
                bool alive = true;
                if (!kBvh) {
                    const uint32_t k = __float_as_uint(p1.w) & ~kHitBit;
                    const float4 alb = s_scene[3u * k + 1u];
                    const float4 emi = s_scene[3u * k + 2u];
                    L = emi.w != 0.0f ? F3{0.0f + 1.0f * emi.x, 0.0f + 1.0f * emi.y, 0.0f + 1.0f * emi.z}
                                      : F3{0.f, 0.f, 0.f};
                    T = F3{1.0f * alb.x, 1.0f * alb.y, 1.0f * alb.z};
                } else {
                    const uint32_t mat = __float_as_uint(p1.w) & ~kHitBit;
                    const float4 alb = sh_mats[2 * mat + 0];
                    const float4 emi = sh_mats[2 * mat + 1];
                    L = emi.w != 0.0f ? F3{0.0f + 1.0f * emi.x, 0.0f + 1.0f * emi.y, 0.0f + 1.0f * emi.z}
                                      : F3{0.f, 0.f, 0.f};
                    T = F3{1.0f * alb.x, 1.0f * alb.y, 1.0f * alb.z};
                }
                rng = rng_seed(__float_as_uint(p0.w), 0u, 0u, frame);
                if constexpr (kNee) {
                    o = F3{p1.x, p1.y, p1.z};
                    bc = 1u;
                    have = true;
                    nee_hit(F3{p0.x, p0.y, p0.z}, fin0);
                    if (pend) {
                        const float4 p2 = s_px[wave][2][r];
                        dt = F3{p2.x, p2.y, p2.z};
                    }
                    alive = false;
                } else
                if (1u > sp.rr_depth) {
                    const float cp = fmaxf(fmaxf(T.x, T.y), T.z);
                    if (random_float(rng) > cp) alive = false;
                    else T = rr_divide(T, cp);
                }
                if (alive) {
                    const float4 p2 = s_px[wave][2][r];
                    dn = F3{p0.x, p0.y, p0.z};
                    dt = F3{p2.x, p2.y, p2.z};
                    pend = true;
                    o = F3{p1.x, p1.y, p1.z};
                    bc = 1u;
                    have = true;
                }
                if (!kNee) fin0 = !alive;
                }
            }
            finish(fin0);
            next = min(limit, next + (uint32_t)__popcll(m));
            SPT_MARK(accumulate_handout_done);
            if (pend) {
                SPT_MARK(sample);
                const F3 dir = bounce_dir_frame<true>(dn, dt, rng);
                if (kNee && !kInline && snew) {
                    nd = dir;
                } else {
                    d = dir;
                    if (kBvh) {
                        trav_init(tv, d);
                        tdone = false;
                    }
                }
            }
            if (kNee && kBvh && snew) {
                trav_init_shadow(tv, d, smax);
                tdone = false;
            }
            if constexpr (kInline) {
                bool fin_s = false;
                if (shadow) {
                    SPT_MARK(shadow);
                    shadow = false;
                    float bt = smax;
                    uint32_t bk = kMiss;
                    closest_flat<kShape, true>(prims, n_prims, o, nd, bt, bk, (sp.flags & kFlagFastDiv) != 0u, sp.flat_ends,
                                               pair_tab, pair_second);
                    if (!(bt < smax)) {
                        const uint32_t e = ring_entry(q);
                        L = F3{L.x + s_L[wave][0][e], L.y + s_L[wave][1][e], L.z + s_L[wave][2][e]};
                    }
                    if (!after) {
                        have = false;
                        fin_s = true;
                    }
                }
                finish(fin_s);
            }
        }
        if (steps_left == ~0u && lane == 0u) atomicAdd(&totals[kTotStalled], 1ull);
        if (kOrdered && plan.cost && chunk < plan.n[0] && lane == 0u)
            plan.cost[chunk] = (uint16_t)min(65535u, (kBvh && kNee) ? ((steps_init - steps_left) * 4u + titer) >> 2
                                                                    : steps_init - steps_left);
        if (ch_on) {
            uint32_t ap = pix0 + cp;
            if constexpr (kView) {
                if (view_on) ap = __float_as_uint(s_px[wave][2][cp].w);
            }
            float* af = reinterpret_cast<float*>(accum) + 4u * (size_t)ap + c0;
            af[0] = acc.x;
            if (pxs == kMaxChunkShift) af[1] = acc.y;
        } else if (!chmode && lane < npx) {
            uint32_t ap = pix0 + lane;
            if constexpr (kView) {
                if (view_on) ap = __float_as_uint(s_px[wave][2][lane].w);
            }
            accum[ap] = acc;
        }
    }
#ifdef SPT_TIMELINE
    if (lane == 0u) {
        unsigned long long* r = g_tl + 4u * (blockIdx.x * kWaves + wave);
        r[0] = tl_start;
        r[1] = tl_last;
        r[2] = wall_clock64();
        r[3] = tl_chunks | ((unsigned long long)xcc << 32) | ((unsigned long long)tl_pxs << 40) |
               ((unsigned long long)tl_live << 48);
    }
#endif
    if (kStats) {
        if (lane == 0u) {
            atomicAdd(&totals[2u * kMaxBounces], (unsigned long long)lane_slots);
            atomicAdd(&totals[2u * kMaxBounces + 1u], (unsigned long long)lane_busy);
        }
        if (kBvh) {
            atomicAdd(&totals[2u * kMaxBounces + 2u], (unsigned long long)bvh_ctr.nodes);
            atomicAdd(&totals[2u * kMaxBounces + 3u], (unsigned long long)bvh_ctr.prims);
        }
        __syncthreads();
        if (threadIdx.x < sp.max_bounces) {
            if (s_seg[threadIdx.x]) atomicAdd(&totals[threadIdx.x], (unsigned long long)s_seg[threadIdx.x]);
            if (s_rmw[threadIdx.x]) atomicAdd(&totals[kMaxBounces + threadIdx.x], (unsigned long long)s_rmw[threadIdx.x]);
        }
        if (kNee && threadIdx.x == 0u && s_shadow[0]) atomicAdd(&totals[kTotShadow], (unsigned long long)s_shadow[0]);
        if constexpr (kPairs != 0u)
            if (threadIdx.x == 0u && *pair_second) atomicAdd(&totals[kTotPairSecond], (unsigned long long)*pair_second);
        if constexpr (kCountSpheres)
            if (threadIdx.x == 0u && pair_second[1]) atomicAdd(&totals[kTotSphereSecond], (unsigned long long)pair_second[1]);
    }
}

__device__ __forceinline__ uint32_t to_u8(float v, float frames) {
    float c = v / frames;
    c = c < 0.0f ? 0.0f : (1.0f < c ? 1.0f : c);
    if (c != c) c = 0.0f;
    return (uint32_t)(uint8_t)(c * 255.0f);
}

__device__ __forceinline__ uint32_t to_u8(float v, float frames, float exposure) {
    float c = v / frames;
    c = c * exposure;
    c = c < 0.0f ? 0.0f : (1.0f < c ? 1.0f : c);
    if (c != c) c = 0.0f;
    return (uint32_t)(uint8_t)(c * 255.0f);
}

__device__ __forceinline__ uint32_t rgba8(float4 a, float frames, float exposure) {
    return (to_u8(a.x, frames, exposure) << 24) | (to_u8(a.y, frames, exposure) << 16) |
           (to_u8(a.z, frames, exposure) << 8) | to_u8(a.w, frames);
}

constexpr uint32_t kFrameBvhBatch = 24;
constexpr uint32_t kFrameBvhBatchLds = 64;

template <bool kStats, bool kBvh, int kEnv, uint64_t kShape = 0, bool kSmall = false, int kNee = 0, bool kRgba = false,
          bool kBsdf = false>
__global__ __launch_bounds__(kBlock, kSmall ? kFrameWavesSmall : (kBvh ? kPathsWavesBvh : kPathsWaves)) void k_frame(const float4* __restrict__ prims, const float4* __restrict__ mats,
                                                  const float4* __restrict__ nodes, uint32_t n_prims,
                                                  float4* __restrict__ accum,
                                                  unsigned long long* __restrict__ totals,
                                                  uint32_t* __restrict__ work, uint32_t* __restrict__ work_next,
                                                  ShadeParams sp, CameraParams cam, NeeParams nee) {
    bake_config<kShape>(sp);
    if (blockIdx.x == 0u && threadIdx.x < kWorkHeads) work_next[threadIdx.x * kWorkStride] = 0u;
    const bool lists = cam.hit_mode == 3u;
    const uint32_t sky_blocks = lists ? cam.sky_blocks : 0u;
    if (blockIdx.x < sky_blocks) {
        const uint32_t n_sky = __builtin_amdgcn_readfirstlane(cam.list_counts[1]);
        for (uint32_t i = blockIdx.x * kBlock + threadIdx.x; i < n_sky; i += sky_blocks * kBlock) {
            const uint32_t px = cam.sky_pix[i];
            const CameraRay cr = camera_ray<kShape, false>(cam, px);
            float4 a = accum[px];
            F3 lc{0.f, 0.f, 0.f};
            if (sp.sky_enabled) {
                const F3 sky = sky_radiance<kEnv>(sp, cr.d);
                lc = F3{0.0f + 1.0f * sky.x, 0.0f + 1.0f * sky.y, 0.0f + 1.0f * sky.z};
            }
            a.x = a.x + lc.x;
// ... 609 lines not shown

void launch_shade(const PassParams& p, uint32_t bounce, hipStream_t s) { launch_shade_kernel(p, bounce, false, s); }
void launch_bounce(const PassParams& p, uint32_t bounce, hipStream_t s) { launch_shade_kernel(p, bounce, true, s); }

void launch_trace_tail(const PassParams& p, uint32_t bounce, hipStream_t s) {
    const ShadeParams sp = shade_params(p, bounce);
    const QueueBufs& cur = p.q[bounce & 1u];
    with_bools(
        [&](auto bvh, auto nee, auto bsdf) {
            k_trace_tail<bvh(), nee(), bsdf()><<<p.n_sub, kBlock, 0, s>>>(p.prims, p.nodes, p.n_prims, p.mats, cur, p.radiance, p.counts, sp, p.n_sub, p.nee);
        },
        p.nodes != nullptr, p.nee.n_emit != 0u, p.bsdf != 0u);
}

__global__ __launch_bounds__(128) void k_chunk_order(const uint16_t* __restrict__ cost, uint32_t n,
                                                     uint32_t* __restrict__ order) {
    constexpr uint32_t kB = 64u, kT = 128u;
    __shared__ uint32_t h[kB][kT];
    __shared__ uint32_t mx[kT];
    const uint32_t t = threadIdx.x;
    const uint32_t per = (n + kT - 1u) / kT, b0 = min(n, t * per), b1 = min(n, b0 + per);
    uint32_t m = 1u;
    for (uint32_t i = b0; i < b1; ++i) m = max(m, (uint32_t)cost[i]);
    mx[t] = m;
    for (uint32_t b = 0; b < kB; ++b) h[b][t] = 0u;
    __syncthreads();
    if (t == 0u) {
        uint32_t v = 1u;
        for (uint32_t u = 0; u < kT; ++u) v = max(v, mx[u]);
        mx[0] = v;
    }
    __syncthreads();
    const uint32_t top = mx[0];
    auto bucket = [&](uint32_t c) { return kB - 1u - min(kB - 1u, (c * kB) / (top + 1u)); };
    for (uint32_t i = b0; i < b1; ++i) h[bucket(cost[i])][t] += 1u;
    __syncthreads();
    if (t == 0u) {
        uint32_t run = 0;
        for (uint32_t b = 0; b < kB; ++b)
            for (uint32_t u = 0; u < kT; ++u) {
                const uint32_t v = h[b][u];
                h[b][u] = run;
                run += v;
            }
    }
    __syncthreads();
    for (uint32_t i = b0; i < b1; ++i) order[h[bucket(cost[i])][t]++] = i;
}

namespace {
template <class K>
const void* kp(K* kernel) {
    return (const void*)kernel;
}

const void* paths_kernel(const PathsVariant& v) {
    const bool env = v.env == 1;
    if (v.bsdf) {
        if (v.env != 2 || v.simd_waves || v.chan || v.jitter || v.nee == kNeeNoSpheres) return nullptr;
        if (!v.bvh) {
            if (v.nee) return v.stats ? kp(k_paths<true, false, 2, 0, 0, false, kNeeAll, false, true>) : kp(k_paths<false, false, 2, 0, 0, false, kNeeAll, false, true>);
            return v.stats ? kp(k_paths<true, false, 2, 0, 0, false, 0, false, true>) : kp(k_paths<false, false, 2, 0, 0, false, 0, false, true>);
        }
        if (v.nee) return v.stats ? kp(k_paths<true, true, 2, 0, 0, false, kNeeAll, false, true>) : kp(k_paths<false, true, 2, 0, 0, false, kNeeAll, false, true>);
        return v.stats ? kp(k_paths<true, true, 2, 0, 0, false, 0, false, true>) : kp(k_paths<false, true, 2, 0, 0, false, 0, false, true>);
    }
    if (v.jitter) {
        if (v.env != 2 || v.simd_waves || v.chan || (!v.bvh && v.nee == kNeeNoSpheres)) return nullptr;
        if (!v.bvh) {
            if (v.nee) return v.stats ? kp(k_paths<true, false, 2, 0, 0, false, kNeeAll, true>) : kp(k_paths<false, false, 2, 0, 0, false, kNeeAll, true>);
            return v.stats ? kp(k_paths<true, false, 2, 0, 0, false, 0, true>) : kp(k_paths<false, false, 2, 0, 0, false, 0, true>);
        }
        if (v.nee == kNeeAll) return v.stats ? kp(k_paths<true, true, 2, 0, 0, false, kNeeAll, true>) : kp(k_paths<false, true, 2, 0, 0, false, kNeeAll, true>);
        if (v.nee) return v.stats ? kp(k_paths<true, true, 2, 0, 0, false, kNeeNoSpheres, true>) : kp(k_paths<false, true, 2, 0, 0, false, kNeeNoSpheres, true>);
        return v.stats ? kp(k_paths<true, true, 2, 0, 0, false, 0, true>) : kp(k_paths<false, true, 2, 0, 0, false, 0, true>);
    }
    if (v.nee) {
        if (v.env != 2 || v.simd_waves || v.chan || (!v.bvh && v.nee != kNeeAll)) return nullptr;
        if (!v.bvh) return v.stats ? kp(k_paths<true, false, 2, 0, 0, false, kNeeAll>) : kp(k_paths<false, false, 2, 0, 0, false, kNeeAll>);
        if (v.nee == kNeeAll) return v.stats ? kp(k_paths<true, true, 2, 0, 0, false, kNeeAll>) : kp(k_paths<false, true, 2, 0, 0, false, kNeeAll>);
        return v.stats ? kp(k_paths<true, true, 2, 0, 0, false, kNeeNoSpheres>) : kp(k_paths<false, true, 2, 0, 0, false, kNeeNoSpheres>);
    }
    if (v.env > 1) return nullptr;
    if (v.simd_waves) {
        if (v.simd_waves != kBvhSmallWaves || !v.bvh || v.stats || v.chan) return nullptr;
        return env ? kp(k_paths<false, true, 1, 0, kBvhSmallWaves>) : kp(k_paths<false, true, 0, 0, kBvhSmallWaves>);
    }
    if (v.chan) {
        if (v.bvh || v.stats) return nullptr;
        return env ? kp(k_paths<false, false, 1, 0, 0, true>) : kp(k_paths<false, false, 0, 0, 0, true>);
    }
    if (v.stats) return v.bvh ? (env ? kp(k_paths<true, true, 1>) : kp(k_paths<true, true, 0>))
                              : (env ? kp(k_paths<true, false, 1>) : kp(k_paths<true, false, 0>));
    return v.bvh ? (env ? kp(k_paths<false, true, 1>) : kp(k_paths<false, true, 0>))
                 : (env ? kp(k_paths<false, false, 1>) : kp(k_paths<false, false, 0>));
}

const void* frame_kernel(const FrameVariant& v) {
    const bool env = v.env == 1;
    if (v.bsdf) {
        if (v.env != 2 || v.small || v.nee == kNeeNoSpheres || (v.rgba && v.stats)) return nullptr;
        if (v.rgba) {
            if (v.nee) return v.bvh ? kp(k_frame<false, true, 2, 0, false, kNeeAll, true, true>) : kp(k_frame<false, false, 2, 0, false, kNeeAll, true, true>);
            return v.bvh ? kp(k_frame<false, true, 2, 0, false, 0, true, true>) : kp(k_frame<false, false, 2, 0, false, 0, true, true>);
        }
        if (v.nee) {
            if (v.bvh) return v.stats ? kp(k_frame<true, true, 2, 0, false, kNeeAll, false, true>) : kp(k_frame<false, true, 2, 0, false, kNeeAll, false, true>);
            return v.stats ? kp(k_frame<true, false, 2, 0, false, kNeeAll, false, true>) : kp(k_frame<false, false, 2, 0, false, kNeeAll, false, true>);
        }
        if (v.bvh) return v.stats ? kp(k_frame<true, true, 2, 0, false, 0, false, true>) : kp(k_frame<false, true, 2, 0, false, 0, false, true>);
        return v.stats ? kp(k_frame<true, false, 2, 0, false, 0, false, true>) : kp(k_frame<false, false, 2, 0, false, 0, false, true>);
    }
    if (v.nee ? (v.env != 2 || v.small || (!v.bvh && v.nee != kNeeAll)) : v.env > 1) return nullptr;
    if (v.small && (!v.bvh || v.stats)) return nullptr;
    if (v.rgba) {
        if (v.stats) return nullptr;
        if (v.nee == kNeeNoSpheres) return kp(k_frame<false, true, 2, 0, false, kNeeNoSpheres, true>);
        if (v.nee) return v.bvh ? kp(k_frame<false, true, 2, 0, false, kNeeAll, true>) : kp(k_frame<false, false, 2, 0, false, kNeeAll, true>);
        if (v.small) return env ? kp(k_frame<false, true, 1, 0, true, 0, true>) : kp(k_frame<false, true, 0, 0, true, 0, true>);
        return v.bvh ? (env ? kp(k_frame<false, true, 1, 0, false, 0, true>) : kp(k_frame<false, true, 0, 0, false, 0, true>))
                     : (env ? kp(k_frame<false, false, 1, 0, false, 0, true>) : kp(k_frame<false, false, 0, 0, false, 0, true>));
    }
    if (v.nee == kNeeNoSpheres) return v.stats ? kp(k_frame<true, true, 2, 0, false, kNeeNoSpheres>) : kp(k_frame<false, true, 2, 0, false, kNeeNoSpheres>);
    if (v.nee && v.bvh) return v.stats ? kp(k_frame<true, true, 2, 0, false, kNeeAll>) : kp(k_frame<false, true, 2, 0, false, kNeeAll>);
    if (v.nee) return v.stats ? kp(k_frame<true, false, 2, 0, false, kNeeAll>) : kp(k_frame<false, false, 2, 0, false, kNeeAll>);
    if (v.small) return env ? kp(k_frame<false, true, 1, 0, true>) : kp(k_frame<false, true, 0, 0, true>);
    if (v.stats) return v.bvh ? (env ? kp(k_frame<true, true, 1>) : kp(k_frame<true, true, 0>))
                              : (env ? kp(k_frame<true, false, 1>) : kp(k_frame<true, false, 0>));
    return v.bvh ? (env ? kp(k_frame<false, true, 1>) : kp(k_frame<false, true, 0>))
                 : (env ? kp(k_frame<false, false, 1>) : kp(k_frame<false, false, 0>));
}

hipFunction_t jit_kernel(JitKind k, const PassParams& p) {
    return k.kind < 0 ? nullptr : jit_function(k.kind, k.env, p.jit_shape, nullptr, p.jit_wait != 0u);
}
int blocks_per_cu(hipFunction_t fn, const void* kernel, size_t lds) {
    int per_cu = 0;
    const hipError_t occ = fn ? hipModuleOccupancyMaxActiveBlocksPerMultiprocessor(&per_cu, fn, kBlock, lds)
                              : hipOccupancyMaxActiveBlocksPerMultiprocessor(&per_cu, kernel, kBlock, lds);
    return occ != hipSuccess || per_cu < 1 ? 1 : per_cu;
}
bool launch_persistent(hipFunction_t fn, const void* kernel, uint32_t grid, size_t lds, void** args, hipStream_t s) {
    if (fn && hipModuleLaunchKernel(fn, grid, 1, 1, kBlock, 1, 1, (unsigned)lds, s, args, nullptr) == hipSuccess) return true;
    assert(kernel && "no such instantiation");
    (void)hipLaunchKernel(kernel, dim3(grid), dim3(kBlock), args, lds, s);
    return false;
}
}

bool launch_paths(const PassParams& p, bool stats, hipStream_t s, const ViewPlan* view_lists, uint32_t view_half) {
    ShadeParams sp = shade_params(p, 0u);
    CameraParams cam = camera_params(p);
    const bool bvh = p.nodes != nullptr;
    const size_t lds_scene = bvh ? 0 : sizeof(float4) * 3u * p.n_prims + flat_pair_table_bytes(p.jit_shape);
    PathsVariant v = paths_variant(p, stats, kMaxChunkShift);
    hipFunction_t fn = jit_kernel(jit_kind(v, p.jit_shape), p);
    const int per_cu = blocks_per_cu(fn, paths_kernel(v), lds_scene);
    ViewPlan view{};
    if (view_lists && view_lists->live && view_lists_scene(p)) view = *view_lists;
    ChunkPlan plan;
    if (view.live) {
        const ViewChunkPlan vp = make_view_plan(p.shard_pixels, view.n_live, view.n_const, resident_waves(per_cu, p.cu_count),
                                                p.chunks_per_wave, p.px_shift);
        plan = vp.plan;
        view.n_sweep = vp.n_sweep;
    } else {
        plan = make_chunk_plan(p.shard_pixels, resident_waves(per_cu, p.cu_count), p.chunks_per_wave, p.px_shift);
    }
    bool record = false;
    const uint64_t order_key = view.live ? view_order_key(plan, view.n_live, view_half) : chunk_order_key(plan, p.shard_pixels);
    if (!p.px_shift && p.chunk_cost && p.chunk_order && plan.n[0] > 1u) {
        if (*p.chunk_order_key == order_key) {
            plan.order = p.chunk_order;
        } else {
            plan.cost = p.chunk_cost;
            record = true;
        }
    }
    v = paths_variant(p, stats, plan.shift[0]);
    if (v.chan) fn = jit_kernel(jit_kind(v, p.jit_shape), p);
    const uint32_t grid = paths_grid(plan, bvh, per_cu, p.cu_count, view.n_sweep);
    void* args[] = {(void*)&p.prims, (void*)&p.mats, (void*)&p.nodes, (void*)&p.n_prims, (void*)&p.accum, (void*)&p.totals,
                    (void*)&p.work, (void*)&p.work_next, &sp, &cam, (void*)&p.n_frames, &plan, (void*)&p.nee, &view};
    const bool specialized = launch_persistent(fn, paths_kernel(v), grid, lds_scene, args, s);
    if (record) {
        k_chunk_order<<<1, 128, 0, s>>>(p.chunk_cost, plan.n[0], p.chunk_order);
        if (hipPeekAtLastError() == hipSuccess) *p.chunk_order_key = order_key;
    }
    return specialized;
}

bool launch_frame(const PassParams& p, bool stats, hipStream_t s) {
    ShadeParams sp = shade_params(p, 0u);
    CameraParams cam = camera_params(p);
    const FrameVariant v = frame_variant(p, stats);
    const size_t lds_scene = v.bvh ? (v.small ? sizeof(uint2) * kBlock * std::max(1u, p.stack_need) : 0)
                                   : sizeof(float4) * 3u * p.n_prims;
    const hipFunction_t fn = jit_kernel(jit_kind(v, p.jit_shape), p);
    FrameVariant asked = v;
    asked.rgba = false;
    const int per_cu = blocks_per_cu(fn, frame_kernel(asked), lds_scene);
    const FrameGrid g = frame_grid(p.shard_pixels, p.live_pixels, p.hit_mode, v.bvh, per_cu, p.cu_count);
    cam.sky_blocks = g.sky_blocks;
    void* args[] = {(void*)&p.prims, (void*)&p.mats, (void*)&p.nodes, (void*)&p.n_prims, (void*)&p.accum, (void*)&p.totals,
                    (void*)&p.work, (void*)&p.work_next, &sp, &cam, (void*)&p.nee};
    return launch_persistent(fn, frame_kernel(v), g.path_grid + g.sky_blocks, lds_scene, args, s);
}

void launch_accumulate(const PassParams& p, hipStream_t s) {
    uint32_t blocks = (p.shard_pixels + kBlock - 1) / kBlock;
    if (blocks > 8192) blocks = 8192;
    if (blocks < 2 * p.max_bounces) blocks = 2 * p.max_bounces;
    if (blocks < 1) blocks = 1;
    k_accumulate<<<blocks, kBlock, 0, s>>>(p);
}

void launch_hit_lists(const PassParams& p, uint32_t* block_scratch, hipStream_t s) {
    const uint32_t n = p.shard_pixels, nb = (n + kBlock - 1u) / kBlock;
    if (n == 0u) return;
    k_hit_count<<<nb, kBlock, 0, s>>>(p.hit_cache, n, block_scratch);
    k_hit_scan<<<1, 1024, 0, s>>>(block_scratch, nb, n, const_cast<uint32_t*>(p.list_counts));
    k_hit_scatter<<<nb, kBlock, 0, s>>>(p.hit_cache, n, block_scratch, const_cast<uint4*>(p.live_rec),
                                        const_cast<uint32_t*>(p.sky_pix));
}

void launch_view_lists(const PassParams& p, float4* live, float4* constant, uint32_t* counts, uint32_t* block_scratch,
                       hipStream_t s) {
    const uint32_t n = p.shard_pixels, nb = (n + kBlock - 1u) / kBlock;
    if (n == 0u) return;
    const ShadeParams sp = shade_params(p, 0u);
    const CameraParams cam = camera_params(p);
    k_view_lists<false><<<nb, kBlock, 0, s>>>(p.prims, p.mats, p.n_prims, sp, cam, block_scratch, live, constant);
    k_hit_scan<<<1, 1024, 0, s>>>(block_scratch, nb, n, counts);
    k_view_lists<true><<<nb, kBlock, 0, s>>>(p.prims, p.mats, p.n_prims, sp, cam, block_scratch, live, constant);
}

void launch_resolve(const float4* accum, uint32_t n, float frames, float exposure, uint32_t* out, hipStream_t s) {
    if (n == 0) return;
    k_resolve<<<(n + kBlock - 1) / kBlock, kBlock, 0, s>>>(accum, n, frames, exposure, out);
}

#ifdef SPT_TIMELINE
extern "C" int spt_exp_timeline(void* out, size_t bytes) {
    if (bytes > sizeof(g_tl)) bytes = sizeof(g_tl);
    if (hipDeviceSynchronize() != hipSuccess) return -1;
    return hipMemcpyFromSymbol(out, HIP_SYMBOL(g_tl), bytes, 0, hipMemcpyDeviceToHost) == hipSuccess ? 0 : -1;
}
#endif
void launch_assemble_rows(const float4* gathered, float4* out, uint32_t width, uint32_t height, uint32_t world,
                          uint32_t rows_max, hipStream_t s) {
    const uint32_t n = width * height;
    if (n == 0) return;
    k_assemble_rows<<<(n + kBlock - 1) / kBlock, kBlock, 0, s>>>(gathered, out, width, height, world, rows_max);
}

void launch_features(const PassParams& p, const uint32_t* mat_map, float4* feat_a, float4* feat_b, float4* albedo,
                     hipStream_t s) {
    const uint32_t n = p.shard_pixels;
    if (n == 0) return;
    const CameraParams cam = camera_params(p);
    const uint32_t nb = (n + kBlock - 1) / kBlock;
    if (p.nodes != nullptr) k_features<true><<<nb, kBlock, 0, s>>>(p.prims, p.mats, p.nodes, p.n_prims, mat_map, cam, feat_a, feat_b, albedo);
    else k_features<false><<<nb, kBlock, 0, s>>>(p.prims, p.mats, p.nodes, p.n_prims, mat_map, cam, feat_a, feat_b, albedo);
}
// ... 5 lines not shown
```

software-path-tracer_amd/csrc/spt_launch_plan.h:

```cpp
#pragma once

#include <algorithm>

#include "spt_jit.h"
#include "spt_kernels.h"

namespace spt {

struct PathsVariant {
    bool stats, bvh;
    int env;
    int simd_waves;
    bool chan;
    int nee;
    bool jitter = false;
    bool bsdf = false;
};
struct FrameVariant {
    bool stats, bvh;
    int env;
    bool small;
    int nee;
    bool rgba;
    bool jitter = false;
    bool bsdf = false;
};

inline int nee_variant(const PassParams& p) {
    if (p.nee.n_emit == 0u) return 0;
    return p.nodes != nullptr && p.nee.spheres == 0u ? kNeeNoSpheres : kNeeAll;
}
inline PathsVariant paths_variant(const PassParams& p, bool stats, uint32_t first_shift) {
    const bool bvh = p.nodes != nullptr;
    const int nee = nee_variant(p);
    PathsVariant v{stats, bvh, nee ? 2 : (p.env ? 1 : 0), 0, false, nee};
    if (p.bsdf) {
        v.env = 2;
        v.nee = nee ? kNeeAll : 0;
        v.bsdf = true;
        return v;
    }
    if (cam_per_path(p.cam_mode)) {
        v.env = 2;
        v.jitter = true;
        return v;
    }
    if (bvh && !stats && !nee && p.n_prims <= kBvhSmall) v.simd_waves = kBvhSmallWaves;
    v.chan = !bvh && !stats && !nee && first_shift < kMaxChunkShift;
    return v;
}
inline FrameVariant frame_variant(const PassParams& p, bool stats) {
    const bool rgba = p.rgba != nullptr;
    stats = stats && !rgba;
    const int nee = nee_variant(p);
    if (p.bsdf) return FrameVariant{stats, p.nodes != nullptr, 2, false, nee ? kNeeAll : 0, rgba, cam_per_path(p.cam_mode), true};
    return FrameVariant{stats, p.nodes != nullptr, nee ? 2 : (p.env ? 1 : 0), frame_small_scene(p, stats), nee, rgba,
                        cam_per_path(p.cam_mode)};
}
inline uint32_t frame_hit_mode(const PassParams& p, bool cache_valid, bool lists) {
    if (cam_per_path(p.cam_mode) || p.bsdf) return 0u;
    return !cache_valid ? 1u : (lists ? 3u : 2u);
}

struct JitKind {
    int kind, env;
};
constexpr JitKind kJitNone{-1, 0};
inline JitKind jit_kind(const PathsVariant& v, uint64_t shape) {
    if (!shape || v.bvh || v.jitter || v.bsdf) return kJitNone;
    if (v.stats) return flat_shape_pairs(shape) ? JitKind{v.nee ? kJitPathsNeeStats : kJitPathsStats, v.env} : kJitNone;
    return JitKind{v.nee ? kJitPathsNee : v.chan ? kJitPathsChan : kJitPaths, v.env};
}
inline JitKind jit_kind(const FrameVariant& v, uint64_t shape) {
    if (!shape || v.bvh || v.stats || v.bsdf) return kJitNone;
    return JitKind{v.rgba ? (v.nee ? kJitFrameNeeRgba : kJitFrameRgba) : (v.nee ? kJitFrameNee : kJitFrame), v.env};
}
struct JitKindList {
    int n;
    JitKind k[3];
};
inline JitKindList jit_kinds_of_scene(bool nee, int env) {
    if (nee) return {2, {{kJitPathsNee, 2}, {kJitFrameNee, 2}}};
    return {3, {{kJitPaths, env}, {kJitFrame, env}, {kJitPathsChan, env}}};
}

inline ChunkPlan make_chunk_plan(uint32_t P, uint32_t resident_waves, uint32_t chunks_per_wave, uint32_t px_shift) {
    ChunkPlan plan{};
    uint32_t s0 = kMaxChunkShift;
    while (s0 > kMinChunkShift && ((uint64_t)P >> s0) < 8ull * resident_waves) --s0;
    if (px_shift) s0 = std::max(kMinChunkShift, std::min(px_shift, kMaxChunkShift));
    const uint32_t s1 = s0 > kMinChunkShift ? s0 - 1u : kMinChunkShift, s2 = s1 > kMinChunkShift ? s1 - 1u : kMinChunkShift;
    plan.shift[0] = s0;
    plan.shift[1] = s1;
    plan.shift[2] = s2;
    if (px_shift || s0 == kMinChunkShift) {
        plan.n[0] = (uint32_t)(((uint64_t)P + (1u << s0) - 1u) >> s0);
        return plan;
    }
    const uint64_t tail = (uint64_t)chunks_per_wave * resident_waves;
    const uint32_t c_px = (uint32_t)std::min<uint64_t>(P, tail << s2);
    const uint32_t b_px = (uint32_t)std::min<uint64_t>(P - c_px, tail << s1) & ~((1u << s1) - 1u);
    const uint32_t a_px = (P - c_px - b_px) & ~((1u << s0) - 1u);
    plan.n[0] = a_px >> s0;
    plan.n[1] = b_px >> s1;
    plan.start[1] = a_px;
    plan.start[2] = a_px + b_px;
    plan.n[2] = (P - a_px - b_px + (1u << s2) - 1u) >> s2;
    return plan;
}
inline uint64_t chunk_order_key(const ChunkPlan& plan, uint32_t P) {
    return ((uint64_t)plan.n[0] << 37) | ((uint64_t)P << 5) | plan.shift[0];
}


#ifndef SPT_VIEW_TIER8
#define SPT_VIEW_TIER8 1
#endif
#ifndef SPT_VIEW_TIER16
#define SPT_VIEW_TIER16 1
#endif
constexpr bool kViewTier8 = SPT_VIEW_TIER8 != 0;
constexpr bool kViewTier16 = SPT_VIEW_TIER16 != 0;
struct ViewChunkPlan {
    ChunkPlan plan;
    uint32_t n_sweep;
};
inline ViewChunkPlan make_view_plan(uint32_t shard_pixels, uint32_t live, uint32_t constant, uint32_t resident_waves,
                                    uint32_t chunks_per_wave, uint32_t px_shift) {
    ViewChunkPlan vp{};
    ChunkPlan& plan = vp.plan;
    vp.n_sweep = (constant + kViewSweep - 1u) / kViewSweep;
    const ChunkPlan pixel_plan = make_chunk_plan(shard_pixels, resident_waves, chunks_per_wave, px_shift);
    const uint32_t s0 = pixel_plan.shift[0], s1 = pixel_plan.shift[1], s2 = pixel_plan.shift[2];
    plan.shift[0] = s0;
    plan.shift[1] = s1;
    plan.shift[2] = s2;
    if (px_shift || s0 == kMinChunkShift) {
        plan.n[0] = (uint32_t)(((uint64_t)live + (1u << s0) - 1u) >> s0);
        return vp;
    }
    const uint64_t tail = shard_pixels ? (uint64_t)chunks_per_wave * resident_waves * live / shard_pixels : 0u;
    const uint32_t c_px = kViewTier8 ? (uint32_t)std::min<uint64_t>(live, tail << s2) : 0u;
    const uint32_t b_px = kViewTier16 ? (uint32_t)std::min<uint64_t>(live - c_px, tail << s1) & ~((1u << s1) - 1u) : 0u;
    const uint32_t a_px = (live - c_px - b_px) & ~((1u << s0) - 1u);
    plan.n[0] = a_px >> s0;
    plan.n[1] = b_px >> s1;
    plan.start[1] = a_px;
    plan.start[2] = a_px + b_px;
    plan.n[2] = (live - a_px - b_px + (1u << s2) - 1u) >> s2;
    return vp;
}
inline uint64_t view_order_key(const ChunkPlan& plan, uint32_t live, uint32_t half = 0u) {
    return (chunk_order_key(plan, live) & ~(3ull << 61)) | ((uint64_t)(half & 3u) << 61) | (1ull << 63);
}

struct ViewSplit {
    uint32_t live_at[3];
    uint32_t const_at[3];
};
inline uint32_t split_cut(uint32_t n, uint32_t unit) {
    unit = std::max(unit, 1u);
    const uint64_t cut = ((uint64_t)n / 2u + unit / 2u) / unit * unit;
    return (uint32_t)std::min<uint64_t>(cut, n);
}
inline ViewSplit make_view_split(uint32_t n_live, uint32_t n_const, uint32_t first_tier_px) {
    return ViewSplit{{0u, split_cut(n_live, first_tier_px), n_live}, {0u, split_cut(n_const, kViewSweep), n_const}};
}
constexpr uint64_t kSplitMinLiveFrames = 1ull << 24;
inline bool split_call_wanted(int32_t knob, uint32_t n_live, uint32_t call_frames, uint32_t max_launch_frames) {
    if (knob) return knob > 0;
    return (uint64_t)n_live * std::min(call_frames, max_launch_frames) >= kSplitMinLiveFrames;
}
inline bool view_half_empty(const ViewSplit& s, uint32_t h) {
    return s.live_at[h + 1] == s.live_at[h] && s.const_at[h + 1] == s.const_at[h];
}

constexpr uint32_t kBlockWaves = kBlock / 64u;
inline uint32_t resident_waves(int per_cu, uint32_t cu_count) { return (uint32_t)per_cu * cu_count * kBlockWaves; }
inline uint32_t paths_grid(const ChunkPlan& plan, bool bvh, int per_cu, uint32_t cu_count, uint32_t sweep_units = 0u) {
    const uint32_t chunks = plan.n[0] + plan.n[1] + plan.n[2] + sweep_units;
    const uint32_t needed = (chunks + kBlockWaves - 1u) / kBlockWaves;
    if (bvh) per_cu = std::min<int>(per_cu, (int)(kMaxResidentWaves / kBlockWaves));
    return std::min<uint32_t>(needed, (uint32_t)per_cu * cu_count);
}

constexpr uint32_t kFrameRunsPerWave = 4;
constexpr uint32_t kFrameListsRpw = 2;
struct FrameGrid {
    uint32_t path_grid, sky_blocks;
};
inline FrameGrid frame_grid(uint32_t shard_pixels, uint32_t live_pixels, uint32_t hit_mode, bool bvh, int per_cu,
                            uint32_t cu_count) {
    const bool lists = hit_mode == 3u;
    const uint32_t units = lists ? live_pixels : shard_pixels;
    const uint32_t runs = (units + frame_chunk(bvh) - 1u) / frame_chunk(bvh);
    if (!bvh) {
        const uint32_t rule_runs = lists ? (shard_pixels + frame_chunk(bvh) - 1u) / frame_chunk(bvh) : runs;
        const uint32_t rpw = lists ? kFrameListsRpw : kFrameRunsPerWave;
        const uint32_t want_blocks = rule_runs / (rpw * kBlockWaves);
        per_cu = std::max(1, std::min(per_cu, (int)((want_blocks + cu_count / 2u) / std::max(1u, cu_count))));
    }
    const uint32_t needed = (runs + kBlockWaves - 1u) / kBlockWaves;
    if (bvh) per_cu = std::min<int>(per_cu, (int)(kMaxResidentWaves / kBlockWaves));
    const uint32_t n_sky = lists ? shard_pixels - live_pixels : 0u;
    return FrameGrid{std::max(1u, std::min<uint32_t>(needed, (uint32_t)per_cu * cu_count)),
                     (n_sky + kBlock * kFrameSkyPerLane - 1u) / (kBlock * kFrameSkyPerLane)};
}

}
```

Baseline: 131,000.

## Add wide 64-pixel chunk variant of flat view-list paths kernel

New measurement: 134,500 (median of 6 runs). +2.7%, better.

```diff
diff --git a/include/spt.h b/include/spt.h
--- a/include/spt.h
+++ b/include/spt.h
@@ -217,6 +217,7 @@
 int spt_set_profiling(spt_ctx* ctx, int mode);
 int spt_get_stats(spt_ctx* ctx, spt_stats* out);
 int spt_stats_clear(spt_ctx* ctx);
+int spt_get_view_wide(spt_ctx* ctx, uint64_t* view_wide);
 
 #define SPT_COMM_ID_BYTES 128
 int spt_comm_available(void);
@@ -240,6 +241,7 @@
     int32_t specialize;
     int32_t view_cache;
     int32_t split_streams;
+    int32_t wide_chunks;
 } spt_tuning;
 int spt_set_tuning(spt_ctx* ctx, const spt_tuning* tuning);
 
diff --git a/software-path-tracer_amd/__init__.py b/software-path-tracer_amd/__init__.py
--- a/software-path-tracer_amd/__init__.py
+++ b/software-path-tracer_amd/__init__.py
@@ -139,12 +139,14 @@
         ("view_split", ctypes.c_uint64),
         ("flat_sphere_second_passes", ctypes.c_uint64),
     ]
+    view_wide = 0
 
     def as_dict(self) -> dict:
         d = {}
         for k, _ in self._fields_:
             v = getattr(self, k)
             d[k] = list(v) if isinstance(v, ctypes.Array) else v
+        d["view_wide"] = self.view_wide
         return d
 
 
@@ -153,7 +155,7 @@
     "spt_set_scene", "spt_configure", "spt_reset", "spt_get_frame_count", "spt_render", "spt_synchronize",
     "spt_shard_pixels", "spt_read_accum", "spt_accum_device_ptr", "spt_copy_accum_device", "spt_resolve_rgba8",
     "spt_resolve_rgba8_exposure", "spt_register_host_output", "spt_render_resolve_rgba8", "spt_assemble_rows",
-    "spt_set_profiling", "spt_get_stats", "spt_stats_clear", "spt_build_scene",
+    "spt_set_profiling", "spt_get_stats", "spt_get_view_wide", "spt_stats_clear", "spt_build_scene",
     "spt_set_env_map", "spt_env_octa_from_equirect",
     "spt_comm_available", "spt_comm_unique_id", "spt_comm_init", "spt_gather_image", "spt_gather_image_overlapped", "spt_gather_wait",
     "spt_comm_destroy", "spt_set_tuning",
@@ -182,6 +184,7 @@
         ("specialize", ctypes.c_int32),
         ("view_cache", ctypes.c_int32),
         ("split_streams", ctypes.c_int32),
+        ("wide_chunks", ctypes.c_int32),
     ]
 
     def __init__(self, **kw):
@@ -253,6 +256,7 @@
         "spt_set_env_map": ([P, P, U32, U32], I),
         "spt_env_octa_from_equirect": ([P, U32, U32, P, U32, U32], I),
         "spt_get_stats": ([P, ctypes.POINTER(SptStats)], I),
+        "spt_get_view_wide": ([P, ctypes.POINTER(ctypes.c_uint64)], I),
         "spt_stats_clear": ([P], I),
         "spt_build_scene": ([U32, P, ctypes.POINTER(U32), P, ctypes.POINTER(U32), ctypes.POINTER(SptEnv)], I),
         "spt_comm_available": ([], I),
@@ -714,6 +718,9 @@
     def stats(self) -> SptStats:
         s = SptStats()
         self._check(self.lib.spt_get_stats(self.h, ctypes.byref(s)), "spt_get_stats")
+        wide = ctypes.c_uint64(0)
+        self._check(self.lib.spt_get_view_wide(self.h, ctypes.byref(wide)), "spt_get_view_wide")
+        s.view_wide = int(wide.value)
         return s
 
     def clear_stats(self) -> None:
diff --git a/software-path-tracer_amd/csrc/spt_capi.hip b/software-path-tracer_amd/csrc/spt_capi.hip
--- a/software-path-tracer_amd/csrc/spt_capi.hip
+++ b/software-path-tracer_amd/csrc/spt_capi.hip
@@ -78,6 +78,8 @@
     bool stream_dirty = true;
     int32_t split_streams = 0;
     bool last_view_split = false;
+    bool last_view_wide = false;
+    int32_t wide_chunks = 0;
     bool accum_shared = false;
     std::string err;
     uint32_t cu_count = 256;
@@ -534,10 +536,14 @@
     return SPT_OK;
 }
 
+static bool wide_possible_ctx(const spt_ctx* c) {
+    return c->view_cache >= 0 && c->px_shift == 0u && wide_possible(c->wide_chunks, c->pixels, c->cfg.shard_count, c->cu_count);
+}
+
 static void prefetch_flat(const spt_ctx* c) {
     if (!(c->has_scene && c->configured && c->n_prims && c->n_nodes == 0 && c->specialize == 0)) return;
     const uint64_t key = flat_jit_key(c);
-    const JitKindList kinds = jit_kinds_of_scene(nee_active(c), c->d_env ? 1 : 0);
+    const JitKindList kinds = jit_kinds_of_scene(nee_active(c), c->d_env ? 1 : 0, wide_possible_ctx(c));
     for (int i = 0; i < kinds.n; ++i) jit_prefetch(kinds.k[i].kind, kinds.k[i].env, key);
 }
 
@@ -1094,8 +1100,8 @@
     return true;
 }
 
-static int launch_paths_split(spt_ctx* c, PassParams p, const ViewPlan& whole, bool launched[2]) {
-    const ViewSplit sp = make_view_split(whole.n_live, whole.n_const, 1u << kMaxChunkShift);
+static int launch_paths_split(spt_ctx* c, PassParams p, const ViewPlan& whole, bool launched[2], int wide) {
+    const ViewSplit sp = make_view_split(whole.n_live, whole.n_const, wide ? kWidePx : 1u << kMaxChunkShift);
     EventPair span_ev;
     if (c->profiling && c->span && begin_persistent(c, span_ev) != SPT_OK) return SPT_ERR_HIP;
     if (c->stream_dirty || c->accum_shared) {
@@ -1124,7 +1130,7 @@
             ++n_ev;
             if (hipEventRecord(ev[n_ev - 1].a, vh.stream) != hipSuccess) rc = fail(c, SPT_ERR_HIP, "k_paths (split): hipEventRecord");
         }
-        c->last_specialized = launch_paths(p, c->counters, vh.stream, &view, h + 1u);
+        c->last_specialized = launch_paths(p, c->counters, vh.stream, &view, h + 1u, wide, &c->last_view_wide);
         launched[h] = true;
         const hipError_t le = hipGetLastError();
         if (le != hipSuccess) {
@@ -1165,7 +1171,9 @@
 static int render_persistent(spt_ctx* c, PassParams& p, uint32_t first_frame, uint32_t n_frames, bool launched[2]) {
     uint32_t done = 0;
     while (done < n_frames) {
-        const uint32_t f = std::min(kPersistentMaxFrames, n_frames - done);
+        const bool view_now = c->view_cache >= 0 && c->view_valid && view_lists_scene(p);
+        const int wide = view_now ? wide_call(c->wide_chunks, wide_eligible(p), wide_first_tier(c->pixels, c->cu_count), c->view_n[0], n_frames) : 0;
+        const uint32_t f = std::min(wide ? kWideMaxFrames : kPersistentMaxFrames, n_frames - done);
         p.first_frame = first_frame + done;
         p.n_frames = f;
         p.n_paths = f * c->pixels;
@@ -1174,7 +1182,7 @@
         const bool view_on = view_scene && c->view_valid;
         if (view_on && split_call_wanted(c->split_streams, c->view_n[0], n_frames, kPersistentMaxFrames) && half_buffers(c)) {
             c->last_view_cached = c->last_view_split = true;
-            const int rc = launch_paths_split(c, p, view, launched);
+            const int rc = launch_paths_split(c, p, view, launched, wide);
             if (rc != SPT_OK) return rc;
             done += f;
             c->passes++;
@@ -1188,7 +1196,7 @@
         p.chunk_cost = c->chunk_cost;
         p.chunk_order = c->chunk_order;
         p.chunk_order_key = &c->chunk_order_key;
-        c->last_specialized = launch_paths(p, c->counters, on_stream(c), view_on ? &view : nullptr);
+        c->last_specialized = launch_paths(p, c->counters, on_stream(c), view_on ? &view : nullptr, 0u, wide, &c->last_view_wide);
         c->last_pairs = c->last_specialized ? flat_shape_pairs(p.jit_shape) : 0u;
         c->last_view_cached = view_on;
         const hipError_t le = hipGetLastError();
@@ -1951,6 +1959,12 @@
     return SPT_OK;
 }
 
+int spt_get_view_wide(spt_ctx* c, uint64_t* view_wide) {
+    if (!c || !view_wide) return SPT_ERR_INVALID;
+    *view_wide = c->last_view_wide ? 1u : 0u;
+    return SPT_OK;
+}
+
 int spt_stats_clear(spt_ctx* c) {
     if (!c) return SPT_ERR_INVALID;
     SPT_HIP(c, hipSetDevice(c->device));
@@ -1974,7 +1988,7 @@
     SPT_HIP(c, hipSetDevice(c->device));
     const uint64_t key = flat_jit_key(c);
     std::string err;
-    const JitKindList kinds = jit_kinds_of_scene(nee_active(c), c->d_env ? 1 : 0);
+    const JitKindList kinds = jit_kinds_of_scene(nee_active(c), c->d_env ? 1 : 0, wide_possible_ctx(c));
     for (int i = 0; i < kinds.n; ++i)
         if (!jit_function(kinds.k[i].kind, kinds.k[i].env, key, &err))
             return fail(c, SPT_ERR_HIP, ("specialized kernels unavailable (the generic ones run): " + err).c_str());
@@ -2015,7 +2029,7 @@
     if (t->chunks_per_wave > 1024 || t->subqueues > 65536 || t->tail_bounce > kMaxBounces ||
         t->bvh_max_leaf > kBvhMaxLeaf || (t->bvh_bins && (t->bvh_bins < 2 || t->bvh_bins > 64)) ||
         t->specialize < -1 || t->specialize > 1 || t->view_cache < -1 || t->view_cache > 0 || t->split_streams < -1 ||
-        t->split_streams > 1)
+        t->split_streams > 1 || t->wide_chunks < -1 || t->wide_chunks > 1)
         return fail(c, SPT_ERR_INVALID, "spt_tuning: value out of range");
     SPT_HIP(c, hipSetDevice(c->device));
     SPT_HIP(c, hipStreamSynchronize(on_stream(c)));
@@ -2043,6 +2057,7 @@
     c->specialize = t->specialize;
     c->view_cache = t->view_cache;
     c->split_streams = t->split_streams;
+    c->wide_chunks = t->wide_chunks;
     return SPT_OK;
 }
 
diff --git a/software-path-tracer_amd/csrc/spt_jit.h b/software-path-tracer_amd/csrc/spt_jit.h
--- a/software-path-tracer_amd/csrc/spt_jit.h
+++ b/software-path-tracer_amd/csrc/spt_jit.h
@@ -9,7 +9,7 @@
 namespace spt {
 
 enum : int { kJitPaths, kJitFrame, kJitPathsChan, kJitPathsNee, kJitFrameNee, kJitFrameRgba, kJitFrameNeeRgba,
-             kJitPathsStats, kJitPathsNeeStats, kJitKinds };
+             kJitPathsStats, kJitPathsNeeStats, kJitPathsWide, kJitPathsWideStats, kJitKinds };
 constexpr int kJitCallersEnv = -1;
 struct JitKindRow {
     const char* kernel;
@@ -27,6 +27,8 @@
     {"k_frame", ", false, 1, true", 2},
     {"k_paths", "", kJitCallersEnv, true},
     {"k_paths", ", 0, false, 1", 2, true},
+    {"k_paths", ", 0, false, 0, false, false, true", kJitCallersEnv},
+    {"k_paths", ", 0, false, 0, false, false, true", kJitCallersEnv, true},
 };
 inline std::string jit_name_expr(int kind, int env, uint64_t shape) {
     const JitKindRow& k = kJitKindTable[kind];
diff --git a/software-path-tracer_amd/csrc/spt_kernels.h b/software-path-tracer_amd/csrc/spt_kernels.h
--- a/software-path-tracer_amd/csrc/spt_kernels.h
+++ b/software-path-tracer_amd/csrc/spt_kernels.h
@@ -165,6 +165,9 @@
 constexpr uint32_t kBvhSmall = 256u * 1024u;
 constexpr uint32_t kMaxChunkShift = 5;
 constexpr uint32_t kMinChunkShift = 0;
+constexpr uint32_t kWideShift = 6;
+constexpr uint32_t kWidePx = 1u << kWideShift;
+constexpr uint32_t kWideMaxFrames = 512;
 
 struct ChunkPlan {
     uint32_t n[3];
@@ -201,7 +204,7 @@
 void launch_trace_tail(const PassParams& p, uint32_t bounce, hipStream_t s);
 void launch_accumulate(const PassParams& p, hipStream_t s);
 bool launch_paths(const PassParams& p, bool stats, hipStream_t s, const ViewPlan* view = nullptr,
-                  uint32_t view_half = 0u);
+                  uint32_t view_half = 0u, int wide_call = 0, bool* ran_wide = nullptr);
 inline bool view_lists_scene(const PassParams& p) {
     return p.nodes == nullptr && p.n_prims != 0u && !cam_per_path(p.cam_mode) && p.bsdf == 0u;
 }
diff --git a/software-path-tracer_amd/csrc/spt_kernels.hip b/software-path-tracer_amd/csrc/spt_kernels.hip
--- a/software-path-tracer_amd/csrc/spt_kernels.hip
+++ b/software-path-tracer_amd/csrc/spt_kernels.hip
@@ -1259,7 +1259,7 @@
 }
 
 template <bool kStats, bool kBvh, int kEnv, uint64_t kShape = 0, int kSimdWaves = 0, bool kChan = false, int kNee = 0,
-          bool kJitter = false, bool kBsdf = false>
+          bool kJitter = false, bool kBsdf = false, bool kWide = false>
 __global__ __launch_bounds__(kBlock, kSimdWaves ? kSimdWaves : (kBvh ? kPathsWavesBvh : ((kNee || kBsdf) ? kPathsWaves : kPathsWavesFlat))) void k_paths(const float4* __restrict__ prims, const float4* __restrict__ mats,
                                                   const float4* __restrict__ nodes, uint32_t n_prims,
                                                   float4* __restrict__ accum,
@@ -1270,14 +1270,16 @@
     constexpr uint32_t kWaves = kBlock / 64u;
     constexpr bool kStart0 = kJitter || kBsdf;
     constexpr bool kView = !kBvh && !kStart0;
+    static_assert(!kWide || (kView && !kChan && !kNee), "the wide form: the flat pixel-lane kernel over a view's lists");
     bake_config<kShape>(sp);
     constexpr uint32_t kRingSlots = ring_slots<kBvh>();
     extern __shared__ float4 s_scene[];
     constexpr uint32_t kPxRecs = kBvh ? 3u : kFlatPxRecs;
-    __shared__ float4 s_px[kWaves][kPxRecs][1u << kMaxChunkShift];
+    constexpr uint32_t kR2 = kWide ? 0u : 2u;
+    __shared__ float4 s_px[kWaves][kWide ? 2u : kPxRecs][kWide ? kWidePx : 1u << kMaxChunkShift];
     __shared__ float s_L[kWaves][3][kRingSlots];
     __shared__ __attribute__((aligned(16))) uint32_t s_cnt[kWaves][64];
-    __shared__ uint8_t s_pix[kWaves][1u << kMaxChunkShift];
+    __shared__ uint8_t s_pix[kWaves][kWide ? 1u : 1u << kMaxChunkShift];
     constexpr uint32_t kTop = kBvh ? (kSimdWaves == 8 ? kBvhTopNodes8 : kBvhTopNodes) : 0u;
     __shared__ float4 s_top[kTop ? 4u * kTop : 1u];
     const uint32_t n_top = min(kTop, sp.n_nodes);
@@ -1311,9 +1313,9 @@
     uint32_t lane_slots = 0, lane_busy = 0;
     BvhCounters bvh_ctr;
     uint32_t n_chunks = plan.n[0] + plan.n[1] + plan.n[2];
-    bool view_on = false;
+    bool view_on = kWide;
     if constexpr (kView) {
-        view_on = view.live != nullptr;
+        if (!kWide) view_on = view.live != nullptr;
         if (view_on) n_chunks += view.n_sweep;
     }
     const uint32_t xcc = xcc_id();
@@ -1423,14 +1425,14 @@
             }
         }
         if (kStats && !kStart0 && lane == 0u) atomicAdd(&s_seg[0], n_frames * npx);
-        const uint32_t live_mask = (uint32_t)__ballot(live_px);
-        const uint32_t n_live = (uint32_t)__popc(live_mask);
+        const uint32_t live_mask = kWide ? 0u : (uint32_t)__ballot(live_px);
+        const uint32_t n_live = kWide ? npx : (uint32_t)__popc(live_mask);
 #ifdef SPT_TIMELINE
         tl_pxs = pxs;
         tl_live = n_live;
 #endif
         if (kOrdered && plan.cost && n_live == 0u && chunk < plan.n[0] && lane == 0u) plan.cost[chunk] = 0u;
-        if (n_live == 0u) {
+        if (!kWide && n_live == 0u) {
             const float lx = __shfl(lc.x, (int)cp, 64), ly = __shfl(lc.y, (int)cp, 64), lz = __shfl(lc.z, (int)cp, 64);
             const float v0 = c0 == 0u ? lx : (c0 == 1u ? ly : lz);
             const float v1 = c0 + 1u == 1u ? ly : lz;
@@ -1447,14 +1449,22 @@
             continue;
         }
         const uint32_t li = __builtin_amdgcn_mbcnt_lo(live_mask, 0u);
+        [[maybe_unused]] const float4* const wrec = kWide ? view.live + 3u * (size_t)pix0 : nullptr;
+        if constexpr (kWide) {
+            if (lane < npx) {
+                s_px[wave][0][lane] = ps.r0;
+                s_px[wave][1][lane] = ps.r1;
+            }
+        } else {
         if (live_px) {
             s_px[wave][0][li] = ps.r0;
             s_px[wave][1][li] = ps.r1;
-            s_px[wave][2][li] = ps.r2;
+            s_px[wave][kR2][li] = ps.r2;
         } else if (lane < npx) {
             s_px[wave][0][n_live + lane - li] = make_float4(lc.x, lc.y, lc.z, 0.f);
         }
         if (lane < px) s_pix[wave][lane] = (uint8_t)(live_px ? li : (kConstPx | (n_live + lane - li)));
+        }
         s_cnt[wave][lane] = 0;
         uint8_t* const ring_flg = reinterpret_cast<uint8_t*>(&s_cnt[wave][0]);
         const uint32_t m_live = __builtin_amdgcn_readfirstlane((0x80000000u + n_live - 1u) / n_live);
@@ -1513,6 +1523,29 @@
                 run += (uint32_t)__builtin_ctz((uint32_t)__builtin_amdgcn_readlane((int)miss, (int)dz)) >> 3;
             const uint32_t k = min(div_live(n_slots - oldest_s), div_live(run - (oldest_s & 3u)));
             if (k == 0u) return;
+            if constexpr (kWide) {
+                if (lane < npx) {
+                    uint32_t e = oldest_s + lane;
+                    uint32_t f = 0;
+                    for (; f + 2u <= k; f += 2u) {
+                        const uint32_t e0 = e & (kRingSlots - 1u), e1 = (e + n_live) & (kRingSlots - 1u);
+                        e += 2u * n_live;
+                        const float x0 = s_L[wave][0][e0], y0 = s_L[wave][1][e0], z0 = s_L[wave][2][e0];
+                        const float x1 = s_L[wave][0][e1], y1 = s_L[wave][1][e1], z1 = s_L[wave][2][e1];
+                        acc.x = (acc.x + x0) + x1;
+                        acc.y = (acc.y + y0) + y1;
+                        acc.z = (acc.z + z0) + z1;
+                        acc.w = (acc.w + 1.0f) + 1.0f;
+                    }
+                    if (f < k) {
+                        const uint32_t e0 = e & (kRingSlots - 1u);
+                        acc.x = acc.x + s_L[wave][0][e0];
+                        acc.y = acc.y + s_L[wave][1][e0];
+                        acc.z = acc.z + s_L[wave][2][e0];
+                        acc.w = acc.w + 1.0f;
+                    }
+                }
+            } else
             if (ch_on) {
                 const uint32_t ix = s_pix[wave][cp];
                 const bool lv = ix < kConstPx;
@@ -1784,6 +1817,8 @@
                     }
                 } else {
                 const float4 p1 = s_px[wave][1][r];
+                float4 p2w = make_float4(0.f, 0.f, 0.f, 0.f);
+                if constexpr (kWide) p2w = wrec[3u * r + 2u];
                 bool alive = true;
                 if (!kBvh) {
                     const uint32_t k = __float_as_uint(p1.w) & ~kHitBit;
@@ -1807,7 +1842,7 @@
                     have = true;
                     nee_hit(F3{p0.x, p0.y, p0.z}, fin0);
                     if (pend) {
-                        const float4 p2 = s_px[wave][2][r];
+                        const float4 p2 = s_px[wave][kR2][r];
                         dt = F3{p2.x, p2.y, p2.z};
                     }
                     alive = false;
@@ -1818,7 +1853,7 @@
                     else T = rr_divide(T, cp);
                 }
                 if (alive) {
-                    const float4 p2 = s_px[wave][2][r];
+                    const float4 p2 = kWide ? p2w : s_px[wave][kR2][r];
                     dn = F3{p0.x, p0.y, p0.z};
                     dt = F3{p2.x, p2.y, p2.z};
                     pend = true;
@@ -1877,7 +1912,7 @@
         if (ch_on) {
             uint32_t ap = pix0 + cp;
             if constexpr (kView) {
-                if (view_on) ap = __float_as_uint(s_px[wave][2][cp].w);
+                if (view_on) ap = __float_as_uint(s_px[wave][kR2][cp].w);
             }
             float* af = reinterpret_cast<float*>(accum) + 4u * (size_t)ap + c0;
             af[0] = acc.x;
@@ -1885,7 +1920,7 @@
         } else if (!chmode && lane < npx) {
             uint32_t ap = pix0 + lane;
             if constexpr (kView) {
-                if (view_on) ap = __float_as_uint(s_px[wave][2][lane].w);
+                if (view_on) ap = __float_as_uint(kWide ? wrec[3u * lane + 2u].w : s_px[wave][kR2][lane].w);
             }
             accum[ap] = acc;
         }
@@ -2661,6 +2696,11 @@
         return v.stats ? kp(k_paths<true, true, 2, 0, 0, false, kNeeNoSpheres>) : kp(k_paths<false, true, 2, 0, 0, false, kNeeNoSpheres>);
     }
     if (v.env > 1) return nullptr;
+    if (v.wide) {
+        if (v.bvh || v.simd_waves || v.chan) return nullptr;
+        if (v.stats) return env ? kp(k_paths<true, false, 1, 0, 0, false, 0, false, false, true>) : kp(k_paths<true, false, 0, 0, 0, false, 0, false, false, true>);
+        return env ? kp(k_paths<false, false, 1, 0, 0, false, 0, false, false, true>) : kp(k_paths<false, false, 0, 0, 0, false, 0, false, false, true>);
+    }
     if (v.simd_waves) {
         if (v.simd_waves != kBvhSmallWaves || !v.bvh || v.stats || v.chan) return nullptr;
         return env ? kp(k_paths<false, true, 1, 0, kBvhSmallWaves>) : kp(k_paths<false, true, 0, 0, kBvhSmallWaves>);
@@ -2727,7 +2767,8 @@
 }
 }
 
-bool launch_paths(const PassParams& p, bool stats, hipStream_t s, const ViewPlan* view_lists, uint32_t view_half) {
+bool launch_paths(const PassParams& p, bool stats, hipStream_t s, const ViewPlan* view_lists, uint32_t view_half,
+                  int wide_call, bool* ran_wide) {
     ShadeParams sp = shade_params(p, 0u);
     CameraParams cam = camera_params(p);
     const bool bvh = p.nodes != nullptr;
@@ -2738,9 +2779,13 @@
     ViewPlan view{};
     if (view_lists && view_lists->live && view_lists_scene(p)) view = *view_lists;
     ChunkPlan plan;
+    bool wide = false;
     if (view.live) {
-        const ViewChunkPlan vp = make_view_plan(p.shard_pixels, view.n_live, view.n_const, resident_waves(per_cu, p.cu_count),
-                                                p.chunks_per_wave, p.px_shift);
+        const uint32_t waves = resident_waves(per_cu, p.cu_count);
+        wide = view.n_live != 0u && p.n_frames <= kWideMaxFrames && wide_eligible(p) &&
+               wide_launch(wide_call, make_chunk_plan(p.shard_pixels, waves, p.chunks_per_wave, p.px_shift).shift[0]);
+        const uint32_t cpw = wide && view_half && !p.chunks_per_wave ? kWideSplitChunksPerWave : p.chunks_per_wave;
+        const ViewChunkPlan vp = make_view_plan(p.shard_pixels, view.n_live, view.n_const, waves, cpw, p.px_shift, wide);
         plan = vp.plan;
         view.n_sweep = vp.n_sweep;
     } else {
@@ -2756,9 +2801,10 @@
             record = true;
         }
     }
-    v = paths_variant(p, stats, plan.shift[0]);
-    if (v.chan) fn = jit_kernel(jit_kind(v, p.jit_shape), p);
-    const uint32_t grid = paths_grid(plan, bvh, per_cu, p.cu_count, view.n_sweep);
+    v = paths_variant(p, stats, plan.shift[0], wide);
+    if (v.chan || v.wide) fn = jit_kernel(jit_kind(v, p.jit_shape), p);
+    if (ran_wide) *ran_wide = v.wide;
+    const uint32_t grid = paths_grid(plan, bvh, v.wide ? blocks_per_cu(fn, paths_kernel(v), lds_scene) : per_cu, p.cu_count, view.n_sweep);
     void* args[] = {(void*)&p.prims, (void*)&p.mats, (void*)&p.nodes, (void*)&p.n_prims, (void*)&p.accum, (void*)&p.totals,
                     (void*)&p.work, (void*)&p.work_next, &sp, &cam, (void*)&p.n_frames, &plan, (void*)&p.nee, &view};
     const bool specialized = launch_persistent(fn, paths_kernel(v), grid, lds_scene, args, s);
diff --git a/software-path-tracer_amd/csrc/spt_launch_plan.h b/software-path-tracer_amd/csrc/spt_launch_plan.h
--- a/software-path-tracer_amd/csrc/spt_launch_plan.h
+++ b/software-path-tracer_amd/csrc/spt_launch_plan.h
@@ -15,6 +15,7 @@
     int nee;
     bool jitter = false;
     bool bsdf = false;
+    bool wide = false;
 };
 struct FrameVariant {
     bool stats, bvh;
@@ -30,7 +31,7 @@
     if (p.nee.n_emit == 0u) return 0;
     return p.nodes != nullptr && p.nee.spheres == 0u ? kNeeNoSpheres : kNeeAll;
 }
-inline PathsVariant paths_variant(const PassParams& p, bool stats, uint32_t first_shift) {
+inline PathsVariant paths_variant(const PassParams& p, bool stats, uint32_t first_shift, bool wide = false) {
     const bool bvh = p.nodes != nullptr;
     const int nee = nee_variant(p);
     PathsVariant v{stats, bvh, nee ? 2 : (p.env ? 1 : 0), 0, false, nee};
@@ -47,6 +48,8 @@
     }
     if (bvh && !stats && !nee && p.n_prims <= kBvhSmall) v.simd_waves = kBvhSmallWaves;
     v.chan = !bvh && !stats && !nee && first_shift < kMaxChunkShift;
+    v.wide = wide && !bvh && !nee;
+    if (v.wide) v.chan = false;
     return v;
 }
 inline FrameVariant frame_variant(const PassParams& p, bool stats) {
@@ -68,6 +71,10 @@
 constexpr JitKind kJitNone{-1, 0};
 inline JitKind jit_kind(const PathsVariant& v, uint64_t shape) {
     if (!shape || v.bvh || v.jitter || v.bsdf) return kJitNone;
+    if (v.wide) {
+        if (v.stats) return flat_shape_pairs(shape) ? JitKind{kJitPathsWideStats, v.env} : kJitNone;
+        return JitKind{kJitPathsWide, v.env};
+    }
     if (v.stats) return flat_shape_pairs(shape) ? JitKind{v.nee ? kJitPathsNeeStats : kJitPathsStats, v.env} : kJitNone;
     return JitKind{v.nee ? kJitPathsNee : v.chan ? kJitPathsChan : kJitPaths, v.env};
 }
@@ -77,10 +84,11 @@
 }
 struct JitKindList {
     int n;
-    JitKind k[3];
-};
-inline JitKindList jit_kinds_of_scene(bool nee, int env) {
+    JitKind k[4];
+};
+inline JitKindList jit_kinds_of_scene(bool nee, int env, bool wide = false) {
     if (nee) return {2, {{kJitPathsNee, 2}, {kJitFrameNee, 2}}};
+    if (wide) return {4, {{kJitPaths, env}, {kJitFrame, env}, {kJitPathsChan, env}, {kJitPathsWide, env}}};
     return {3, {{kJitPaths, env}, {kJitFrame, env}, {kJitPathsChan, env}}};
 }
 
@@ -126,12 +134,14 @@
     uint32_t n_sweep;
 };
 inline ViewChunkPlan make_view_plan(uint32_t shard_pixels, uint32_t live, uint32_t constant, uint32_t resident_waves,
-                                    uint32_t chunks_per_wave, uint32_t px_shift) {
+                                    uint32_t chunks_per_wave, uint32_t px_shift, bool wide = false) {
     ViewChunkPlan vp{};
     ChunkPlan& plan = vp.plan;
     vp.n_sweep = (constant + kViewSweep - 1u) / kViewSweep;
     const ChunkPlan pixel_plan = make_chunk_plan(shard_pixels, resident_waves, chunks_per_wave, px_shift);
-    const uint32_t s0 = pixel_plan.shift[0], s1 = pixel_plan.shift[1], s2 = pixel_plan.shift[2];
+    wide = wide && !px_shift;
+    const uint32_t s0 = wide ? kWideShift : pixel_plan.shift[0], s1 = wide ? kWideShift - 1u : pixel_plan.shift[1],
+                   s2 = wide ? kWideShift - 2u : pixel_plan.shift[2];
     plan.shift[0] = s0;
     plan.shift[1] = s1;
     plan.shift[2] = s2;
@@ -140,8 +150,9 @@
         return vp;
     }
     const uint64_t tail = shard_pixels ? (uint64_t)chunks_per_wave * resident_waves * live / shard_pixels : 0u;
-    const uint32_t c_px = kViewTier8 ? (uint32_t)std::min<uint64_t>(live, tail << s2) : 0u;
-    const uint32_t b_px = kViewTier16 ? (uint32_t)std::min<uint64_t>(live - c_px, tail << s1) & ~((1u << s1) - 1u) : 0u;
+    const uint64_t cap = wide ? live / 4u : live;
+    const uint32_t c_px = kViewTier8 ? (uint32_t)std::min<uint64_t>(cap, tail << s2) : 0u;
+    const uint32_t b_px = kViewTier16 ? (uint32_t)std::min<uint64_t>(std::min<uint64_t>(cap, live - c_px), tail << s1) & ~((1u << s1) - 1u) : 0u;
     const uint32_t a_px = (live - c_px - b_px) & ~((1u << s0) - 1u);
     plan.n[0] = a_px >> s0;
     plan.n[1] = b_px >> s1;
@@ -163,13 +174,34 @@
     const uint64_t cut = ((uint64_t)n / 2u + unit / 2u) / unit * unit;
     return (uint32_t)std::min<uint64_t>(cut, n);
 }
-inline ViewSplit make_view_split(uint32_t n_live, uint32_t n_const, uint32_t first_tier_px) {
+inline ViewSplit make_view_split(uint32_t n_live, uint32_t n_const, uint32_t first_tier_px = 1u << kMaxChunkShift) {
     return ViewSplit{{0u, split_cut(n_live, first_tier_px), n_live}, {0u, split_cut(n_const, kViewSweep), n_const}};
 }
 constexpr uint64_t kSplitMinLiveFrames = 1ull << 24;
 inline bool split_call_wanted(int32_t knob, uint32_t n_live, uint32_t call_frames, uint32_t max_launch_frames) {
     if (knob) return knob > 0;
     return (uint64_t)n_live * std::min(call_frames, max_launch_frames) >= kSplitMinLiveFrames;
+}
+constexpr uint64_t kWideMinLiveFrames = 3ull << 20;
+constexpr int kWideBlocksPerCu = 7;
+inline bool wide_first_tier(uint32_t shard_pixels, uint32_t cu_count) {
+    return make_chunk_plan(shard_pixels, (uint32_t)kWideBlocksPerCu * cu_count * (kBlock / 64u), 0u, 0u).shift[0] == kMaxChunkShift;
+}
+constexpr uint32_t kWideSplitChunksPerWave = 1;
+inline bool wide_eligible(const PassParams& p) {
+    return view_lists_scene(p) && nee_variant(p) == 0 && p.shard_count <= 1u && p.px_shift == 0u;
+}
+inline int wide_call(int32_t knob, bool eligible, bool first_tier_32, uint32_t n_live, uint32_t call_frames) {
+    if (knob < 0 || !eligible) return 0;
+    if (knob > 0) return 2;
+    return first_tier_32 && (uint64_t)n_live * std::min(call_frames, kWideMaxFrames) >= kWideMinLiveFrames ? 1 : 0;
+}
+inline bool wide_launch(int wide_call, uint32_t pixel_first_shift) {
+    return wide_call == 2 || (wide_call == 1 && pixel_first_shift == kMaxChunkShift);
+}
+inline bool wide_possible(int32_t knob, uint32_t shard_pixels, uint32_t shard_count, uint32_t cu_count) {
+    if (knob < 0 || shard_count > 1u) return false;
+    return knob > 0 || (wide_first_tier(shard_pixels, cu_count) && (uint64_t)shard_pixels * kWideMaxFrames >= kWideMinLiveFrames);
 }
 inline bool view_half_empty(const ViewSplit& s, uint32_t h) {
     return s.live_at[h + 1] == s.live_at[h] && s.const_at[h + 1] == s.const_at[h];
```
